# akanazawa/human_dynamics

Hardware: NVIDIA H100
Metric: frames/sec (ResNet->f_movie->SMPL LBS) (higher is better)
Workload: dtype f32 (wgmma 3x fp16 head/remainder split, fp32 two-level accumulate)

## Files before the change

human_dynamics_b200/_lib.py:

```python
from __future__ import annotations

import ctypes as C
import os

_HERE = os.path.dirname(os.path.abspath(__file__))
LIB_PATH = os.path.join(_HERE, 'libhd_b200.so')

HD_IMPL_SIMT, HD_IMPL_TC_3XTF32, HD_IMPL_TC_1XTF32, HD_IMPL_TC_3XF16, HD_IMPL_TC_1XF16 = 0, 1, 2, 3, 4
HD_CONV_NO_TMA_EPILOGUE = 1
HD_CONV_INPUT_PLANES = 2
HD_PACK_FORWARD, HD_PACK_BACKWARD_DATA = 0, 1
IMPL_BY_NAME = {'simt': HD_IMPL_SIMT, 'tc3': HD_IMPL_TC_3XTF32, 'tc1': HD_IMPL_TC_1XTF32, 'tc3h': HD_IMPL_TC_3XF16,
                'tc1h': HD_IMPL_TC_1XF16}


class ConvDesc(C.Structure):
    _fields_ = [
        ('in_', C.c_void_p), ('in_ld', C.c_longlong),
        ('n_img', C.c_int), ('H', C.c_int), ('W', C.c_int), ('Cin', C.c_int),
        ('Ho', C.c_int), ('Wo', C.c_int), ('KH', C.c_int), ('KW', C.c_int),
        ('stride', C.c_int), ('pad_t', C.c_int), ('pad_l', C.c_int),
        ('w_kn', C.c_void_p), ('w_nk_hi', C.c_void_p), ('w_nk_lo', C.c_void_p),
        ('Cout', C.c_int), ('K_pad', C.c_int),
        ('pre_scale', C.c_void_p), ('pre_shift', C.c_void_p), ('pre_img_stride', C.c_int), ('pre_relu', C.c_int),
        ('post_scale', C.c_void_p), ('post_shift', C.c_void_p), ('post_relu', C.c_int),
        ('res', C.c_void_p), ('res_ld', C.c_longlong), ('res_H', C.c_int), ('res_W', C.c_int), ('res_stride', C.c_int),
        ('out', C.c_void_p), ('out_ld', C.c_longlong),
        ('impl', C.c_int),
        ('tmap_hi', C.c_void_p), ('tmap_lo', C.c_void_p),
        ('in_hi', C.c_void_p), ('in_lo', C.c_void_p),
        ('out_hi', C.c_void_p), ('out_lo', C.c_void_p), ('out2_ld', C.c_longlong),
        ('post2_scale', C.c_void_p), ('post2_shift', C.c_void_p), ('post2_relu', C.c_int),
        ('tmap_res', C.c_void_p), ('tmap_out', C.c_void_p), ('tmap_out_hi', C.c_void_p), ('tmap_out_lo', C.c_void_p),
        ('flags', C.c_int),
        ('tmap_hi_n64', C.c_void_p), ('tmap_lo_n64', C.c_void_p),
        ('out_subsample', C.c_int),
    ]


WEIGHT_FN = C.CFUNCTYPE(C.c_void_p, C.c_void_p, C.c_char_p, C.POINTER(C.c_longlong))


class SmplConsts(C.Structure):
    _fields_ = [
        ('num_verts', C.c_int), ('num_kps', C.c_int), ('lbs_nnz', C.c_int), ('kp_nnz_total', C.c_int),
        ('v_template', C.c_void_p), ('dirs', C.c_void_p), ('J_template', C.c_void_p), ('J_shapedirs', C.c_void_p),
        ('lbs_idx', C.c_void_p), ('lbs_w', C.c_void_p),
        ('kp_ptr', C.c_void_p), ('kp_vidx', C.c_void_p), ('kp_w', C.c_void_p),
        ('parents', C.c_int * 24),
    ]


class SmplGradConsts(C.Structure):
    _fields_ = [
        ('num_verts', C.c_int), ('num_kps', C.c_int), ('num_tiles', C.c_int), ('tile_verts', C.c_int),
        ('kpv_ptr', C.c_void_p), ('kpv_kidx', C.c_void_p), ('kpv_w', C.c_void_p),
        ('lbt_ptr', C.c_void_p), ('lbt_v', C.c_void_p), ('lbt_w', C.c_void_p),
    ]


SMPL_GRAD_TILE, SMPL_GRAD_CLD = 256, 224


class RenderParams(C.Structure):
    _fields_ = [
        ('color', C.c_float * 3), ('light_dir', C.c_float * 3), ('ambient', C.c_float), ('directional', C.c_float),
        ('bg', C.c_float * 3), ('near_z', C.c_float), ('far_z', C.c_float), ('eye_z', C.c_float),
        ('rot', C.c_float * 9), ('use_rot', C.c_int),
    ]


HD_LOSS_KP_L1, HD_LOSS_MSE_ROWS = 0, 1
HD_LOSS_KP_CAMERA, HD_LOSS_KP_OPTCAM, HD_LOSS_KP_RAW = 0, 1, 2
HD_LOSS_MAX_TERMS, HD_LOSS_MAX_GRADS = 64, 16


class LossTerm(C.Structure):
    _fields_ = [
        ('kind', C.c_int), ('proj', C.c_int), ('B', C.c_int), ('Tw', C.c_int), ('p_t0', C.c_int), ('q_t0', C.c_int),
        ('p_T', C.c_int), ('q_T', C.c_int), ('K', C.c_int), ('D', C.c_int),
        ('p', C.c_void_p), ('p_clip', C.c_longlong), ('p_frame', C.c_longlong),
        ('q', C.c_void_p), ('q_clip', C.c_longlong), ('q_frame', C.c_longlong),
        ('cam', C.c_void_p), ('cam_clip', C.c_longlong), ('cam_frame', C.c_longlong),
        ('w', C.c_void_p), ('cam_out', C.c_void_p), ('scale', C.c_float),
    ]


class LossGrad(C.Structure):
    _fields_ = [('src', C.c_void_p), ('grad', C.c_void_p), ('numel', C.c_longlong)]


HD_ADAM_MAX_TENSORS = 256


class AdamTensor(C.Structure):
    _fields_ = [('param', C.c_void_p), ('grad', C.c_void_p), ('m', C.c_void_p), ('v', C.c_void_p), ('numel', C.c_longlong)]


HD_AUG_SRC_U8, HD_AUG_ROTATE, HD_AUG_FLIP = 1, 2, 4


class TubeAugArgs(C.Structure):
    _fields_ = [
        ('frames', C.c_void_p), ('F', C.c_int), ('H', C.c_int), ('W', C.c_int), ('flags', C.c_int),
        ('trans', C.c_void_p), ('scale', C.c_void_p), ('rot', C.c_void_p), ('flip', C.c_void_p),
        ('labels', C.c_void_p), ('K', C.c_int), ('centers', C.c_void_p), ('poses', C.c_void_p), ('gt3ds', C.c_void_p),
        ('S', C.c_int), ('trans_max', C.c_int), ('geom', C.c_void_p),
        ('labels_out', C.c_void_p), ('centers_out', C.c_void_p), ('poses_out', C.c_void_p), ('gt3ds_out', C.c_void_p),
        ('crops', C.c_void_p), ('plane_hi', C.c_void_p), ('plane_lo', C.c_void_p), ('WP', C.c_int),
    ]


HD_EVAL_KP, HD_EVAL_KP_PA, HD_EVAL_KP_PCK, HD_EVAL_JOINTS, HD_EVAL_JOINTS_PA, HD_EVAL_ACCEL, HD_EVAL_ACCEL_ERROR, HD_EVAL_VIS3D = range(8)
HD_EVAL_COLS = 8


class EvalFramesArgs(C.Structure):
    _fields_ = [
        ('N', C.c_int), ('n_seq', C.c_int), ('seq_start', C.c_void_p), ('K', C.c_int), ('J', C.c_int),
        ('kps_gt', C.c_void_p), ('kps_gt_ld', C.c_longlong), ('kps_pred', C.c_void_p), ('kps_pred_ld', C.c_longlong),
        ('joints_gt', C.c_void_p), ('joints_gt_ld', C.c_longlong), ('joints_pred', C.c_void_p), ('joints_pred_ld', C.c_longlong),
        ('img_size', C.c_float), ('min_visible', C.c_int), ('out', C.c_void_p),
    ]


HD_JPEG_BAD_CODE, HD_JPEG_OVERRUN, HD_JPEG_MARKER, HD_JPEG_BAD_HEADER = 1, 2, 4, 8


class JpegHuffman(C.Structure):
    _fields_ = [('bits', C.c_uint8 * 16), ('vals', C.c_uint8 * 256)]


class JpegHeader(C.Structure):
    _fields_ = [
        ('width', C.c_int), ('height', C.c_int), ('h_samp', C.c_int), ('v_samp', C.c_int), ('restart_interval', C.c_int),
        ('qt', C.c_int * 3), ('dc', C.c_int * 3), ('ac', C.c_int * 3), ('data_offset', C.c_longlong), ('data_bytes', C.c_longlong),
    ]


class JpegTables(C.Structure):
    _fields_ = [('quant', (C.c_uint16 * 64) * 4), ('dc', JpegHuffman * 4), ('ac', JpegHuffman * 4),
                ('quant_defined', C.c_int), ('dc_defined', C.c_int), ('ac_defined', C.c_int)]


_vp, _i, _ll, _f, _sz, _ull = C.c_void_p, C.c_int, C.c_longlong, C.c_float, C.c_size_t, C.c_ulonglong
SIGNATURES = {
    'hd_version': (_i, []),
    'hd_status_string': (C.c_char_p, [_i]),
    'hd_last_error': (C.c_char_p, []),
    'hd_launch_count': (_ll, []),
    'hd_launch_count_reset': (None, []),
    'hd_conv_gemm': (_i, [C.POINTER(ConvDesc), _vp]),
    'hd_conv_gemm_profile': (_i, [C.POINTER(ConvDesc), _vp, _vp]),
    'hd_conv_gemm_chain': (_i, [C.POINTER(ConvDesc), C.POINTER(ConvDesc), _vp]),
    'hd_conv_gemm_chain_supported': (_i, [C.POINTER(ConvDesc), C.POINTER(ConvDesc)]),
    'hd_make_weight_tmap': (_i, [_vp, _i, _i, _i, _i, _vp]),
    'hd_make_act_tmap': (_i, [_vp, _ll, _i, _ll, _i, _vp]),
    'hd_pack_conv1_planes': (_i, [_vp, _vp, _vp, _i, _i, _i, _i, _vp]),
    'hd_conv1_7x7s2': (_i, [_vp, _vp, _vp, _vp, _i, _i, _i, _vp]),
    'hd_maxpool3x3s2_same': (_i, [_vp, _vp, _i, _i, _i, _i, _vp, _vp, _vp, _vp, _vp]),
    'hd_subsample': (_i, [_vp, _vp, _i, _i, _i, _i, _i, _vp]),
    'hd_bnrelu_avgpool': (_i, [_vp, _vp, _vp, _vp, _i, _i, _i, _vp]),
    'hd_bn_stats_workspace_bytes': (_sz, [_ll, _i]),
    'hd_bn_batch_stats': (_i, [_vp, _ll, _i, _ll, _vp, _vp, _f] + [_vp] * 6 + [C.c_double, _vp, _sz, _vp]),
    'hd_bn_moving_update': (_i, [_vp, _vp, _ll, _i, C.c_double, _vp, _vp, _vp]),
    'hd_conv_wgrad_workspace_bytes': (_sz, [_ll, _i, _i, _i]),
    'hd_conv_wgrad': (_i, [_vp, _ll] + [_i] * 11 + [_vp, _vp, _vp, _ll, _i, _vp, _vp, _vp, _sz, _vp]),
    'hd_conv_wgrad_ex': (_i, [_vp, _ll] + [_i] * 11 + [_vp, _vp, _vp, _ll, _i, _vp, _vp, _vp, _sz, _i, _vp]),
    'hd_bn_relu_backward_workspace_bytes': (_sz, [_ll, _i]),
    'hd_bn_relu_backward': (_i, [_vp, _vp, _i, _ll, _i, _vp, _vp, _vp, _vp, _f, _vp, _i, _i, _i, _vp, _vp, _vp, _vp, _sz, _vp]),
    'hd_maxpool3x3s2_same_backward': (_i, [_vp, _vp, _vp, _i, _i, _i, _i, _vp]),
    'hd_zero_insert': (_i, [_vp, _vp] + [_i] * 7 + [_vp]),
    'hd_process_image': (_i, [_vp, _i, _i, _i, _vp, _vp, _i, _vp, _vp, _i, _vp]),
    'hd_crop_geometry': (_i, [_i, _i, _vp, _i, _vp, _vp, _vp]),
    'hd_groupnorm_stats': (_i, [_vp, _vp, _vp, _vp, _vp, _i, _i, _i, _i, _f, _vp]),
    'hd_groupnorm_relu_split': (_i, [_vp, _vp, _vp, _vp, _vp, _i, _i, _i, _i, _f, _vp]),
    'hd_split_f16': (_i, [_vp, _vp, _vp, _ll, _vp]),
    'hd_ief_fc1_theta': (_i, [_vp, _vp, _i, _vp, _i, _i, _vp, _vp, _vp, _i, _vp]),
    'hd_ief_fc3': (_i, [_vp, _vp, _vp, _vp, _i, _vp, _i, _i, _i, _i, _vp]),
    'hd_ief_fc1_theta_dropout': (_i, [_vp, _vp, _i, _vp, _i, _i, _vp, _vp, _vp, _i, _ull, _ull, _i, _f, _vp]),
    'hd_ief_fc3_dropout': (_i, [_vp, _vp, _vp, _vp, _i, _vp, _i, _i, _i, _i, _ull, _ull, _i, _f, _vp]),
    'hd_dropout_mask': (_i, [_ull, _ull, _i, _i, _i, _f, _vp, _vp]),
    'hd_ief_delta_init': (_i, [_vp, _vp, _i, _i, _vp]),
    'hd_net_destroy': (None, [_vp]),
    'hd_net_error': (C.c_char_p, [_vp]),
    'hd_net_num_launches': (_ll, [_vp]),
    'hd_resnet50_create': (_i, [_vp, _vp, _i, _i, C.POINTER(_vp)]),
    'hd_resnet50_forward': (_i, [_vp, _vp, _vp, _vp]),
    'hd_fmovie_create': (_i, [_vp, _vp, _i, _i, _i, C.POINTER(_vp)]),
    'hd_fmovie_forward': (_i, [_vp, _vp, _vp, _vp]),
    'hd_ief_create': (_i, [_vp, _vp, _i, C.POINTER(_i), _i, C.POINTER(_vp)]),
    'hd_ief_forward': (_i, [_vp, _vp, _vp, _vp, _vp]),
    'hd_smpl_pack_sizes': (_i, [_i, _i, _vp, _vp, C.POINTER(_i), C.POINTER(_i)]),
    'hd_smpl_pack': (_i, [_i, _i] + [_vp] * 13 + [_i] + [_vp] * 4),
    'hd_smpl_workspace_bytes': (_sz, [_i]),
    'hd_smpl_forward': (_i, [C.POINTER(SmplConsts), _vp, _i, _vp, _i, _i, _vp, _vp, _vp, _vp, _vp, _i, _vp, _i, _i, _vp, _sz, _vp]),
    'hd_smpl_pose': (_i, [C.POINTER(SmplConsts), _vp, _i, _vp, _i, _i, _vp, _vp, _vp, _vp, _i, _vp, _vp, _vp, _vp, _i, _i, _vp, _sz, _vp]),
    'hd_smpl_lbs_tc': (_i, [_vp, _vp, _vp, _vp, _vp, _ll, _vp, _i, _i, _i, _i, _vp]),
    'hd_smpl_lbs': (_i, [C.POINTER(SmplConsts), _vp, _ll, _vp, _vp, _i, _i, _i, _vp]),
    'hd_smpl_joints': (_i, [C.POINTER(SmplConsts), _vp, _vp, _i, _vp, _vp, _i, _i, _i, _vp]),
    'hd_rodrigues': (_i, [_vp, _vp, _i, _vp]),
    'hd_rot2aa': (_i, [_vp, _vp, _i, _vp]),
    'hd_global_rigid': (_i, [_vp, _vp, C.POINTER(C.c_int), _vp, _vp, _i, _i, _vp]),
    'hd_orth_proj': (_i, [_vp, _vp, _vp, _i, _i, _vp]),
    'hd_smpl_backward_workspace_bytes': (_sz, [_i, _i]),
    'hd_smpl_lbs_backward': (_i, [C.POINTER(SmplConsts), C.POINTER(SmplGradConsts), _vp, _ll, _vp, _vp, _vp, _vp, _vp, _i, _vp]),
    'hd_smpl_pose_backward': (_i, [C.POINTER(SmplConsts), _vp, _i, _vp, _i, _i, _vp, _vp, _i, _vp, _vp, _vp, _i, _vp, _i, _vp]),
    'hd_rodrigues_backward': (_i, [_vp, _vp, _vp, _i, _vp]),
    'hd_global_rigid_backward': (_i, [_vp, _vp, C.POINTER(C.c_int), _vp, _vp, _vp, _vp, _i, _i, _vp]),
    'hd_orth_proj_backward': (_i, [_vp, _vp, _vp, _vp, _vp, _i, _i, _vp]),
    'hd_pack_weight': (_i, [_vp, _i, _i, _i, _i, _i, _vp, _vp, _i, _i, _vp]),
    'hd_transpose_split': (_i, [_vp, _ll, _i, _ll, _i, _vp, _vp, _ll, _i, _ll, _vp]),
    'hd_im2col_t': (_i, [_vp, _i, _i, _i, _i, _i, _vp, _vp, _i, _vp, _ll, _ll, _vp]),
    'hd_groupnorm_relu_backward': (_i, [_vp] * 8 + [_i, _i, _i, _i, _f, _i, _vp]),
    'hd_col_sum': (_i, [_vp, _ll, _i, _ll, _vp, _vp]),
    'hd_relu_backward': (_i, [_vp, _vp, _vp, _ll, _vp]),
    'hd_fc_small_dgrad': (_i, [_vp, _i, _vp, _i, _i, _vp, _vp, _i, _vp]),
    'hd_relu_dropout_backward': (_i, [_vp, _vp, _vp, _ll, _f, _vp]),
    'hd_fc_small_dgrad_dropout': (_i, [_vp, _i, _vp, _i, _i, _vp, _f, _vp, _i, _vp]),
    'hd_add_strided': (_i, [_vp, _ll, _vp, _ll, _vp, _ll, _i, _i, _vp]),
    'hd_dpose_workspace_bytes': (_sz, [_i]),
    'hd_dpose_trunk_forward': (_i, [_vp] * 10 + [_i, _vp]),
    'hd_dpose_out_forward': (_i, [_vp] * 4 + [_i, _vp]),
    'hd_dpose_trunk_backward': (_i, [_vp] * 11 + [_sz, _i, _vp]),
    'hd_dpose_grad_reduce': (_i, [_vp, _sz, _i, _vp, _vp]),
    'hd_loss_workspace_bytes': (_sz, [_vp, _i]),
    'hd_loss_forward': (_i, [_vp, _i, _vp, _vp, _sz, _vp]),
    'hd_loss_backward': (_i, [_vp, _i, _vp, _i, _vp, _vp, _sz, _vp]),
    'hd_adam_tf': (_i, [C.POINTER(AdamTensor), _i, _f, _f, _f, _f, _vp, _vp]),
    'hd_render_workspace_bytes': (_sz, [_i, _i, _i]),
    'hd_tube_augment': (_i, [C.POINTER(TubeAugArgs), _vp]),
    'hd_render_mesh': (_i, [_vp, _ll, _i, _i, _vp, _i, _vp, _i, C.POINTER(RenderParams), _vp, _i, _vp, _vp, _vp, _sz, _vp]),
    'hd_eval_frames': (_i, [C.POINTER(EvalFramesArgs), _vp]),
    'hd_eval_mesh_tpose': (_i, [C.POINTER(SmplConsts), _vp, _i, _vp, _i, _i, _vp, _vp]),
    'hd_eval_verts_error': (_i, [_vp, _ll, _vp, _ll, _i, _i, _vp, _vp]),
    'hd_jpeg_parse': (_i, [_vp, _sz, C.POINTER(JpegHeader), C.POINTER(JpegTables)]),
    'hd_jpeg_workspace_bytes': (_sz, [_i, _i, _i, _i, _i]),
    'hd_jpeg_decode': (_i, [_vp, _ll, _vp, _i, _i, _i, _i, _i, _vp, _i, _vp, _i, _vp, _vp, _vp, _sz, _vp]),
}


def _load():
    if not os.path.exists(LIB_PATH):
        raise RuntimeError(
            'human_dynamics_b200: %s is missing -- build it with `make -C human_dynamics_b200/csrc` '
            '(or `python -c "import __graft_entry__ as g; g.build()"`). There is no CPU fallback.' % LIB_PATH)
    lib = C.CDLL(LIB_PATH)
    for name, (res, args) in SIGNATURES.items():
        fn = getattr(lib, name)
        fn.restype = res
        fn.argtypes = args
    return lib


lib = _load()


class HDError(RuntimeError):
    pass


def check(rc: int, what: str = ''):
    if rc != 0:
        raise HDError('%s failed: %s [%s]' % (what or 'libhd_b200 call', lib.hd_status_string(rc).decode(),
                                              lib.hd_last_error().decode()))


def dptr(t, dtype=None):
    import torch
    if t is None:
        return None
    if not isinstance(t, torch.Tensor) or not t.is_cuda:
        raise HDError('expected a CUDA torch.Tensor (no CPU fallback exists), got %r' % (type(t),))
    if dtype is not None and t.dtype != dtype:
        raise HDError('expected dtype %s, got %s' % (dtype, t.dtype))
    return C.c_void_p(t.data_ptr())


def fptr(t):
    import torch
    return dptr(t, torch.float32)


def current_stream():
    import torch
    return C.c_void_p(torch.cuda.current_stream().cuda_stream)
```

human_dynamics_b200/csrc/conv_tc.cu:

```cuda
#include <cuda.h>
#include <cuda_fp16.h>
#include <cstdlib>
#include "conv_common.cuh"
#include "tc_ptx.cuh"

namespace hd {
namespace {

constexpr int BM = 128;
constexpr int BOX_BYTES = 64 * 128;
constexpr int W_PROD = 8;
constexpr int STAGE_OUT = 1, STAGE_PAIR = 2;

using namespace ptx;

template <bool SPLIT, bool HALF, bool ASPLIT, int BN, bool RES = false, bool SHORT = false, bool CM = false>
struct Cfg {
  static_assert(BN == 64 || (BN == 128 && HALF && ASPLIT), "128-wide N tiles: pre-split fp16 path only");
  static_assert(!RES || ASPLIT, "residual by TMA: pre-split fp16 path only");
  static_assert(!SHORT || (BN == 64 && HALF && ASPLIT), "two CTAs per SM: 64-wide pre-split fp16 tiles only");
  static_assert(!CM || (BN == 64 && HALF && ASPLIT && !RES && !SHORT), "channels on M: 64-channel pre-split fp16 tiles, no residual");
  static constexpr int CTAS = SHORT ? 2 : 1;
  static constexpr int TM = CM ? 256 : BM;
  static constexpr int A_BYTES = TM * 128;
  static constexpr int PROD_THREADS = BN == 128 || SHORT || CM ? 128 : 256;
  static constexpr int NUM_THREADS = 256 + PROD_THREADS;
  static constexpr int ROW_STEP = PROD_THREADS / 8;
  static constexpr int ROWS = TM / ROW_STEP;
  static constexpr int PROD_REGS = SHORT ? 32 : CM ? 56 : BN == 128 ? 40 : 104, CONS_REGS = SHORT ? 104 : CM ? 224 : BN == 128 ? 232 : 152;
  static_assert(256 * CONS_REGS + PROD_THREADS * PROD_REGS <= NUM_THREADS * (65536 / (CTAS * NUM_THREADS) / 8 * 8),
                "setmaxnreg split beyond the CTA's registers");
  static constexpr int NACC = CM ? 64 : BN / 2;
  static constexpr int STAGES = SHORT ? 1 : CM ? 2 : BN == 128 ? (RES ? 2 : 3) : (RES ? 3 : 4);
  static constexpr int BKE = HALF ? 64 : 32;
  static constexpr int B_TILE_BYTES = BN * 128;
  static constexpr int B_OFFSET = (SPLIT ? 2 : 1) * A_BYTES;
  static constexpr int STAGE_BYTES = (SPLIT ? 2 : 1) * (A_BYTES + B_TILE_BYTES);
  static constexpr int RES_OFFSET = STAGES * STAGE_BYTES;
  static constexpr int RES_SLOT_BYTES = RES || SHORT ? 64 * BN * 4 : 0;
  static constexpr int STG_OFFSET = SHORT ? RES_OFFSET : RES_OFFSET + 2 * RES_SLOT_BYTES;
  static constexpr int STG_BYTES = ASPLIT ? (CM ? 4 : 2) * BOX_BYTES : 0;
  static_assert(!SHORT || STG_BYTES == RES_SLOT_BYTES, "SHORT: the staging buffer is the residual slot");
  static constexpr int BAR_OFFSET = SHORT ? RES_OFFSET + 2 * RES_SLOT_BYTES : STG_OFFSET + 2 * STG_BYTES;
  static constexpr int SMEM_BYTES = BAR_OFFSET + 128 + 1024;
  static_assert(SMEM_BYTES <= 232448, "dynamic shared memory beyond the 227 KB a CTA can opt into");
  static_assert(CTAS * (SMEM_BYTES + 1024) <= 233472, "CTAS CTAs (and the 1 KB each reserves) beyond an SM's 228 KB");
  static constexpr int PF = HALF ? 2 : 3;
  static constexpr int V = HALF ? 2 : 1;
};

template <bool ADD_R = false>
__device__ __forceinline__ void epi2_rn(float &y0, float &y1, const float *has_sc, float2 sc, const float *has_sh, float2 sh,
                                        const float2 *r, int relu) {
  if (has_sc) { y0 = __fmul_rn(y0, sc.x); y1 = __fmul_rn(y1, sc.y); }
  if (has_sh) { y0 = __fadd_rn(y0, sh.x); y1 = __fadd_rn(y1, sh.y); }
  if (ADD_R) { const float2 v = *r; y0 = __fadd_rn(y0, v.x); y1 = __fadd_rn(y1, v.y); }
  if (relu) { y0 = fmaxf(y0, 0.f); y1 = fmaxf(y1, 0.f); }
}

template <int R>
struct RowState {
  int n[R], iy[R], ix[R];
};

template <bool SPLIT, int PCH, bool HALF, bool GATHER, bool ASPLIT, int BN, bool RES, bool SHORT, bool CM>
__global__ void __launch_bounds__((Cfg<SPLIT, HALF, ASPLIT, BN, RES, SHORT, CM>::NUM_THREADS), (Cfg<SPLIT, HALF, ASPLIT, BN, RES, SHORT, CM>::CTAS))
conv_gemm_tc_kernel(const ConvParams p, const __grid_constant__ CUtensorMap tmap_hi, const __grid_constant__ CUtensorMap tmap_lo,
                    const __grid_constant__ CUtensorMap tmap_res, const __grid_constant__ CUtensorMap tmap_out,
                    const __grid_constant__ CUtensorMap tmap_out_hi, const __grid_constant__ CUtensorMap tmap_out_lo, const int stage) {
  using C = Cfg<SPLIT, HALF, ASPLIT, BN, RES, SHORT, CM>;
  constexpr bool MEM_STAMPS = BN == 128 || SHORT || CM;
  constexpr int BKE = C::BKE, PF = C::PF, V = C::V, STAGES = C::STAGES, R = C::ROWS, RS = C::ROW_STEP, NA = C::NACC;
  extern __shared__ uint8_t smem_raw[];
  const uint32_t smem_base = (smem_u32(smem_raw) + 1023u) & ~1023u;
  uint8_t *smem = smem_raw + (smem_base - smem_u32(smem_raw));
  const uint32_t bar_base = smem_base + C::BAR_OFFSET;
  auto full_bar = [&](int s) { return bar_base + 8u * s; };
  auto empty_bar = [&](int s) { return bar_base + 8u * (STAGES + s); };
  auto res_bar = [&](int g) { return bar_base + 8u * (2 * STAGES + g); };

  const int warp = threadIdx.x >> 5, lane = threadIdx.x & 31;
  const int num_k = (GATHER ? p.K_pad : p.K) / BKE;
  const int tiles_n = (p.Cout + BN - 1) / BN;
  const int num_tiles = ((p.M + C::TM - 1) / C::TM) * tiles_n;
  const int my_tiles = (num_tiles - (int)blockIdx.x + (int)gridDim.x - 1) / (int)gridDim.x;

  if (threadIdx.x == 0) {
    for (int s = 0; s < STAGES; ++s) {
      mbar_init(full_bar(s), ASPLIT ? C::PROD_THREADS + 1 : 9);
      mbar_init(empty_bar(s), 8);
    }
    if (RES) for (int g = 0; g < 2; ++g) mbar_init(res_bar(g), 1);
    asm volatile("fence.mbarrier_init.release.cluster;" ::: "memory");
  }
  __syncthreads();

  if (warp >= W_PROD) {
    asm volatile("setmaxnreg.dec.sync.aligned.u32 %0;" ::"n"(C::PROD_REGS));
    const int t = threadIdx.x - W_PROD * 32;
    const int j = t & 7;
    const int rb = t >> 3;
    const uint32_t sw_off = (uint32_t)((j ^ (rb & 7)) << 4);
    const bool prof = p.dbg != nullptr && blockIdx.x == 0 && t == 0;
    long long t_wait = 0, t_start = prof && !MEM_STAMPS ? clock64() : 0;
    if (MEM_STAMPS && prof) { p.dbg[0] = clock64(); p.dbg[1] = 0; }
    auto wait_empty = [&](int s, uint32_t ph) {
      if (MEM_STAMPS && prof) p.dbg[1] -= clock64();
      const long long tw0 = !MEM_STAMPS && prof ? clock64() : 0;
      mbar_wait(empty_bar(s), ph ^ 1u);
      if (!MEM_STAMPS && prof) t_wait += clock64() - tw0;
      if (MEM_STAMPS && prof) p.dbg[1] += clock64();
    };
    const int total = my_tiles * num_k;
    auto load_b = [&](int s, int ti, int kc) {
      if (t != 0) return;
      const int n0 = (((int)blockIdx.x + ti * (int)gridDim.x) % tiles_n) * BN;
      const uint32_t b_hi = smem_base + s * C::STAGE_BYTES + C::B_OFFSET;
      const int boxes = (BN == 128 && n0 + 64 < p.Cout) ? 2 : 1;
      mbar_arrive_expect_tx(full_bar(s), (SPLIT ? 2 : 1) * boxes * BOX_BYTES);
      for (int b = 0; b < boxes; ++b) {
        tma_load_2d(b_hi + b * BOX_BYTES, &tmap_hi, full_bar(s), kc * BKE, n0 + 64 * b);
        if (SPLIT) tma_load_2d(b_hi + C::B_TILE_BYTES + b * BOX_BYTES, &tmap_lo, full_bar(s), kc * BKE, n0 + 64 * b);
      }
    };

    auto enter_tile = [&](int ti, RowState<R> &rs) {
      const int tile = (int)blockIdx.x + ti * (int)gridDim.x;
      const int m0 = (tile / tiles_n) * C::TM;
      const int hw = p.Ho * p.Wo;
#pragma unroll
      for (int i = 0; i < R; ++i) {
        const int m = m0 + rb + RS * i;
        if (m < p.M) {
          const int n = m / hw;
          const int r = m - n * hw;
          const int oy = r / p.Wo, ox = r - oy * p.Wo;
          rs.n[i] = n; rs.iy[i] = oy * p.stride - p.pad_t; rs.ix[i] = ox * p.stride - p.pad_l;
        } else {
          rs.n[i] = -1; rs.iy[i] = 0; rs.ix[i] = 0;
        }
      }
    };
    if constexpr (ASPLIT) {
      const __half *ihi = reinterpret_cast<const __half *>(p.in_hi);
      const __half *ilo = reinterpret_cast<const __half *>(p.in_lo);
      if (SHORT || (!CM && !p.planes && p.KH * p.KW <= 32 && (long long)p.n_img * p.H * p.W * p.in_ld < (1ll << 31))) {
        const uint32_t off0 = (uint32_t)rb * 128u + sw_off;
        int base[R];
        uint32_t mask[R];
        int kc = 0, ti = 0, tap = 0, ci0 = 0, kx = 0, ky = 0, tap_off = 0;
        for (int q = 0; q < total; ++q) {
          if (kc == 0) {
            const int tile = (int)blockIdx.x + ti * (int)gridDim.x;
            const int m0 = (tile / tiles_n) * C::TM + rb;
            const int hw = p.Ho * p.Wo;
#pragma unroll
            for (int i = 0; i < R; ++i) {
              const int m = m0 + RS * i;
              uint32_t mk = 0;
              int b = 0;
              if (m < p.M) {
                const int n = m / hw;
                const int r = m - n * hw;
                const int oy = r / p.Wo, ox = r - oy * p.Wo;
                const int iy0 = oy * p.stride - p.pad_t, ix0 = ox * p.stride - p.pad_l;
                b = ((n * p.H + iy0) * p.W + ix0) * p.in_ld + j * 8;
                int t = 0;
                for (int yy = 0; yy < p.KH; ++yy)
                  for (int xx = 0; xx < p.KW; ++xx, ++t)
                    if ((unsigned)(iy0 + yy) < (unsigned)p.H && (unsigned)(ix0 + xx) < (unsigned)p.W) mk |= 1u << t;
              }
              base[i] = SHORT && !(mk & 1u) ? -1 : b;
              mask[i] = mk;
            }
            tap = 0; ci0 = 0; kx = 0; ky = 0; tap_off = 0;
          }
          const int s = q % STAGES;
          const uint32_t ph = (uint32_t)(q / STAGES) & 1u;
          wait_empty(s, ph);
          load_b(s, ti, kc);
          const uint32_t a_hi = smem_base + s * C::STAGE_BYTES + off0;
          const int eo = SHORT ? ci0 : tap_off + ci0;
#pragma unroll
          for (int i = 0; i < R; ++i) {
            const bool ok = SHORT ? base[i] >= 0 : (mask[i] >> tap) & 1u;
            const int e = ok ? base[i] + eo : 0;
            cp_async16(a_hi + i * RS * 128, ihi + e, ok ? 16u : 0u);
            if (SPLIT) cp_async16(a_hi + C::A_BYTES + i * RS * 128, ilo + e, ok ? 16u : 0u);
          }
          asm volatile("cp.async.mbarrier.arrive.noinc.shared::cta.b64 [%0];" ::"r"(full_bar(s)) : "memory");
          ci0 += BKE;
          if (ci0 == p.Cin) {
            ci0 = 0; ++tap;
            if (++kx == p.KW) { kx = 0; ++ky; }
            tap_off = (ky * p.W + kx) * p.in_ld;
          }
          if (++kc == num_k) { kc = 0; ++ti; }
        }
      } else if (!SHORT && p.planes && (long long)p.n_img * p.H * p.W * p.in_ld < (1ll << 31)) {
        const uint32_t off0 = (uint32_t)rb * 128u + sw_off;
        const int jt = j >> 2;
        const int row_step = 2 * p.W * (int)p.in_ld;
        int base[R];
        int kc = 0, ti = 0;
        for (int q = 0; q < total; ++q) {
          if (kc == 0) {
            const int tile = (int)blockIdx.x + ti * (int)gridDim.x;
            const int m0 = (tile / tiles_n) * C::TM + rb;
            const int hw = p.Ho * p.Wo;
#pragma unroll
            for (int i = 0; i < R; ++i) {
              const int m = m0 + RS * i;
              int b = -1;
              if (m < p.M) {
                const int n = m / hw;
                const int r = m - n * hw;
                const int oy = r / p.Wo, ox = r - oy * p.Wo;
                b = ((n * p.H + oy * p.stride + jt) * p.W + ox * p.stride) * (int)p.in_ld + (j & 3) * 8;
              }
              base[i] = b;
            }
          }
          const int s = q % STAGES;
          const uint32_t ph = (uint32_t)(q / STAGES) & 1u;
          wait_empty(s, ph);
          load_b(s, ti, kc);
          const uint32_t a_hi = smem_base + s * C::STAGE_BYTES + off0;
          const bool tap_ok = 2 * kc + jt < 7;
          const int eo = kc * row_step;
#pragma unroll
          for (int i = 0; i < R; ++i) {
            const bool ok = tap_ok && base[i] >= 0;
            const int e = ok ? base[i] + eo : 0;
            cp_async16_ca(a_hi + i * RS * 128, ihi + e, ok ? 16u : 0u);
            if (SPLIT) cp_async16_ca(a_hi + C::A_BYTES + i * RS * 128, ilo + e, ok ? 16u : 0u);
          }
          asm volatile("cp.async.mbarrier.arrive.noinc.shared::cta.b64 [%0];" ::"r"(full_bar(s)) : "memory");
          if (++kc == num_k) { kc = 0; ++ti; }
        }
      } else if (!SHORT && !CM) {
      RowState<R> rs;
      int kc = 0, ti = 0;
      for (int q = 0; q < total; ++q) {
        if (kc == 0) enter_tile(ti, rs);
        const int s = q % STAGES;
        const uint32_t ph = (uint32_t)(q / STAGES) & 1u;
        wait_empty(s, ph);
        load_b(s, ti, kc);
        const int kb = kc * BKE;
        const int tap = p.planes ? 2 * kc + (j >> 2) : kb / p.Cin;
        const int ci = p.planes ? (j & 3) * 8 : kb - tap * p.Cin + j * 8;
        const int ky = tap / p.KW, kx = tap - ky * p.KW;
        const bool tap_ok = !p.planes || tap < 7;
        const uint32_t a_hi = smem_base + s * C::STAGE_BYTES, a_lo = a_hi + C::A_BYTES;
#pragma unroll
        for (int i = 0; i < R; ++i) {
          const int iy = rs.iy[i] + ky, ix = rs.ix[i] + kx;
          const bool ok = tap_ok && rs.n[i] >= 0 && iy >= 0 && iy < p.H && ix >= 0 && ix < p.W;
          const size_t e = ok ? ((size_t)((size_t)rs.n[i] * p.H + iy) * p.W + ix) * p.in_ld + ci : 0;
          const uint32_t off = (uint32_t)(rb + RS * i) * 128u + sw_off;
          if (p.planes) {
            cp_async16_ca(a_hi + off, ihi + e, ok ? 16u : 0u);
            if (SPLIT) cp_async16_ca(a_lo + off, ilo + e, ok ? 16u : 0u);
          } else {
            cp_async16(a_hi + off, ihi + e, ok ? 16u : 0u);
            if (SPLIT) cp_async16(a_lo + off, ilo + e, ok ? 16u : 0u);
          }
        }
        asm volatile("cp.async.mbarrier.arrive.noinc.shared::cta.b64 [%0];" ::"r"(full_bar(s)) : "memory");
        if (++kc == num_k) { kc = 0; ++ti; }
      }
      }
      cp_async_commit();
      cp_async_wait<0>();
      if (prof) { p.dbg[0] = clock64() - (MEM_STAMPS ? p.dbg[0] : t_start); if (!MEM_STAMPS) p.dbg[1] = t_wait; }
    } else {
    RowState<R> pf_rs, st_rs;
    float4 ring[PF][4 * V];
    uint32_t vmask[PF];
    int pf_kc = 0, pf_ti = 0;
    auto prefetch = [&](float4 *dst, uint32_t &vm) {
      if (pf_kc == 0) enter_tile(pf_ti, pf_rs);
      if (GATHER) {
        const int seg = p.KW * p.Cin, segp = (seg + 7) & ~7;
        const int g8 = (pf_kc * BKE + j * (4 * V)) / 8;
        const int gpr = segp >> 3;
        const int ky = g8 / gpr, r0 = (g8 - ky * gpr) * 8;
        vm = 0;
#pragma unroll
        for (int i = 0; i < 4; ++i) {
          const int iy = pf_rs.iy[i] + ky;
          const bool okr = pf_rs.n[i] >= 0 && ky < p.KH && iy >= 0 && iy < p.H;
          const int c0 = pf_rs.ix[i] * p.Cin + r0;
          const float *src = p.in + ((size_t)((size_t)(okr ? pf_rs.n[i] : 0) * p.H + (okr ? iy : 0)) * p.W) * p.in_ld + c0;
          const int rowlen = p.W * p.Cin;
          float xs[8];
#pragma unroll
          for (int e = 0; e < 8; ++e) {
            const bool ok = okr && (r0 + e) < seg && (c0 + e) >= 0 && (c0 + e) < rowlen;
            xs[e] = ok ? __ldg(src + e) : 0.f;
          }
          dst[i * V] = make_float4(xs[0], xs[1], xs[2], xs[3]);
          dst[i * V + V - 1] = make_float4(xs[4], xs[5], xs[6], xs[7]);
          if (pf_rs.n[i] >= 0) vm |= 1u << i;
        }
        if (++pf_kc == num_k) { pf_kc = 0; ++pf_ti; }
        return;
      }
      const int kb = pf_kc * BKE;
      const int tap = kb / p.Cin, ci = kb - tap * p.Cin + j * (4 * V);
      const int ky = tap / p.KW, kx = tap - ky * p.KW;
      vm = 0;
#pragma unroll
      for (int i = 0; i < 4; ++i) {
        const int iy = pf_rs.iy[i] + ky, ix = pf_rs.ix[i] + kx;
        const bool ok = pf_rs.n[i] >= 0 && (unsigned)iy < (unsigned)p.H && (unsigned)ix < (unsigned)p.W;
        if (ok) {
          const float4 *src = reinterpret_cast<const float4 *>(p.in + ((size_t)((size_t)pf_rs.n[i] * p.H + iy) * p.W + ix) * p.in_ld + ci);
#pragma unroll
          for (int v = 0; v < V; ++v) dst[i * V + v] = __ldg(src + v);
          vm |= 1u << i;
        } else {
#pragma unroll
          for (int v = 0; v < V; ++v) dst[i * V + v] = make_float4(0.f, 0.f, 0.f, 0.f);
        }
      }
      if (++pf_kc == num_k) { pf_kc = 0; ++pf_ti; }
    };
    int st_kc = 0, st_ti = 0;
    auto consume = [&](int q, float4 *cur, uint32_t vm) {
      if (st_kc == 0) enter_tile(st_ti, st_rs);
      const int s = q % STAGES;
      const uint32_t ph = (uint32_t)(q / STAGES) & 1u;
      long long tw0 = prof ? clock64() : 0;
      mbar_wait(empty_bar(s), ph ^ 1u);
      if (prof) t_wait += clock64() - tw0;
      load_b(s, st_ti, st_kc);
      uint8_t *a_hi = smem + s * C::STAGE_BYTES;
      uint8_t *a_lo = a_hi + C::A_BYTES;
      const int pci = p.pre_scale ? (st_kc * BKE) % p.Cin + j * (4 * V) : 0;
#pragma unroll
      for (int i = 0; i < 4; ++i) {
        float xs[4 * V];
#pragma unroll
        for (int v = 0; v < V; ++v) {
          const float4 x = cur[i * V + v];
          xs[4 * v] = x.x; xs[4 * v + 1] = x.y; xs[4 * v + 2] = x.z; xs[4 * v + 3] = x.w;
        }
        if (p.pre_scale && (vm & (1u << i))) {
          const size_t po = (size_t)(p.pre_img_stride != 0 ? st_rs.n[i] : 0) * p.pre_img_stride + pci;
#pragma unroll
          for (int v = 0; v < V; ++v) {
            const float4 sc = __ldg(reinterpret_cast<const float4 *>(p.pre_scale + po) + v);
            const float4 sh = __ldg(reinterpret_cast<const float4 *>(p.pre_shift + po) + v);
            xs[4 * v] = xs[4 * v] * sc.x + sh.x; xs[4 * v + 1] = xs[4 * v + 1] * sc.y + sh.y;
            xs[4 * v + 2] = xs[4 * v + 2] * sc.z + sh.z; xs[4 * v + 3] = xs[4 * v + 3] * sc.w + sh.w;
          }
          if (p.pre_relu) {
#pragma unroll
            for (int e = 0; e < 4 * V; ++e) xs[e] = fmaxf(xs[e], 0.f);
          }
        }
        uint32_t h[4], l[4];
        if (!HALF) {
#pragma unroll
          for (int e = 0; e < 4; ++e) {
            const float hf = rn_tf32(xs[e]);
            h[e] = __float_as_uint(hf);
            l[e] = __float_as_uint(rn_tf32(xs[e] - hf));
          }
        } else {
#pragma unroll
          for (int e = 0; e < 4; ++e) split_f16x2(xs[2 * e], xs[2 * e + 1], h[e], l[e]);
        }
        const uint32_t off = (uint32_t)(rb + 32 * i) * 128u + sw_off;
        *reinterpret_cast<uint4 *>(a_hi + off) = make_uint4(h[0], h[1], h[2], h[3]);
        if (SPLIT) *reinterpret_cast<uint4 *>(a_lo + off) = make_uint4(l[0], l[1], l[2], l[3]);
      }
      asm volatile("fence.proxy.async.shared::cta;" ::: "memory");
      __syncwarp();
      if (lane == 0) mbar_arrive(full_bar(s));
      if (++st_kc == num_k) { st_kc = 0; ++st_ti; }
    };
#pragma unroll
    for (int u = 0; u < PF - 1; ++u)
      if (u < total) prefetch(ring[u], vmask[u]);
    for (int q0 = 0; q0 < total; q0 += PF) {
#pragma unroll
      for (int u = 0; u < PF; ++u) {
        const int q = q0 + u;
        if (q < total) {
          if (q + PF - 1 < total) prefetch(ring[(u + PF - 1) % PF], vmask[(u + PF - 1) % PF]);
          consume(q, ring[u], vmask[u]);
        }
      }
    }
    if (prof) { p.dbg[0] = clock64() - t_start; p.dbg[1] = t_wait; }
    }
  } else if (warp < W_PROD) {
    asm volatile("setmaxnreg.inc.sync.aligned.u32 %0;" ::"n"(C::CONS_REGS));
    const int wg = warp >> 2;
    const bool prof = p.dbg != nullptr && blockIdx.x == 0 && threadIdx.x == 0;
    long long t_wait = 0, t_start = prof && !MEM_STAMPS && !RES ? clock64() : 0;
    if ((RES || MEM_STAMPS) && prof) p.dbg[2] = clock64();
    if (prof) { p.dbg[3] = 0; p.dbg[4] = 0; p.dbg[5] = 0; p.dbg[6] = 0; }
    const int hw = p.Ho * p.Wo;
    const int frow = wg * 64 + (warp & 3) * 16 + (lane >> 2);
    const int fcol = 2 * (lane & 3);
    float acc[NA], accx[SPLIT ? NA : 1], sums_[SHORT ? 1 : NA];
    float *const sums = SHORT ? acc : sums_;
#pragma unroll
    for (int i = 0; i < NA; ++i) {
      acc[i] = 0.f;
      if constexpr (SPLIT) accx[i] = 0.f;
    }
    uint8_t *res_sm = smem + C::RES_OFFSET + wg * C::RES_SLOT_BYTES;
    const bool res_issuer = RES && (threadIdx.x & 127) == 0;
    const bool stg_issuer = ASPLIT && (threadIdx.x & 127) == 0;
    auto load_res = [&](int ti) {
      const int tile = (int)blockIdx.x + ti * (int)gridDim.x;
      const int r0 = (tile / tiles_n) * BM + 64 * wg, c0 = (tile % tiles_n) * BN;
      const int cols = p.Cout - c0 < BN ? p.Cout - c0 : BN;
      const int boxes = r0 < p.M ? (cols + 31) / 32 : 0;
      const uint32_t slot = smem_base + C::RES_OFFSET + wg * C::RES_SLOT_BYTES;
      mbar_arrive_expect_tx(res_bar(wg), boxes * (64 * 128));
      for (int b = 0; b < boxes; ++b) tma_load_2d(slot + b * (64 * 128), &tmap_res, res_bar(wg), c0 + 32 * b, r0);
    };
    if (res_issuer && my_tiles > 0) load_res(0);
    int q = 0;
    for (int ti = 0; ti < my_tiles; ++ti) {
      if (!SHORT) {
#pragma unroll
        for (int i = 0; i < NA; ++i) sums[i] = 0.f;
      }
      for (int kc = 0; kc < num_k; ++kc, ++q) {
        const int s = q % STAGES;
        const uint32_t ph = (uint32_t)(q / STAGES) & 1u;
        const bool group_start = (kc % PCH) == 0;
        if (MEM_STAMPS && prof) p.dbg[3] -= clock64();
        const long long tw0 = !MEM_STAMPS && prof ? clock64() : 0;
        mbar_wait(full_bar(s), ph);
        if (!MEM_STAMPS && prof) t_wait += clock64() - tw0;
        if (MEM_STAMPS && prof) p.dbg[3] += clock64();
        if (ASPLIT) asm volatile("fence.proxy.async.shared::cta;" ::: "memory");
        const uint32_t a_hi = smem_base + s * C::STAGE_BYTES + wg * (C::TM / 2 * 128);
        const uint32_t a_lo = a_hi + C::A_BYTES;
        const uint32_t b_hi = smem_base + s * C::STAGE_BYTES + C::B_OFFSET;
        const uint32_t b_lo = b_hi + C::B_TILE_BYTES;
        const uint64_t da_hi = make_smem_desc(a_hi), da_lo = make_smem_desc(a_lo);
        const uint64_t db_hi = make_smem_desc(b_hi), db_lo = make_smem_desc(b_lo);
        fence_regs(acc);
        if constexpr (SPLIT) fence_regs(accx);
        wgmma_fence();
#pragma unroll
        for (int k = 0; k < 4; ++k) {
          const uint64_t adv = (uint64_t)((k * 32) >> 4);
          if constexpr (CM) {
            if constexpr (SPLIT) {
              wgmma_m64n128k16_f16(accx, db_hi + adv, da_lo + adv, (kc | k) != 0);
              wgmma_m64n128k16_f16(accx, db_lo + adv, da_hi + adv, 1u);
            }
            wgmma_m64n128k16_f16(acc, db_hi + adv, da_hi + adv, !(group_start && k == 0));
          } else if constexpr (BN == 128) {
            if constexpr (SPLIT) {
              wgmma_m64n128k16_f16(accx, da_lo + adv, db_hi + adv, (kc | k) != 0);
              wgmma_m64n128k16_f16(accx, da_hi + adv, db_lo + adv, 1u);
            }
            wgmma_m64n128k16_f16(acc, da_hi + adv, db_hi + adv, !(group_start && k == 0));
          } else if constexpr (HALF) {
            if constexpr (SPLIT) {
              wgmma_m64n64k16_f16(accx, da_lo + adv, db_hi + adv, (kc | k) != 0);
              wgmma_m64n64k16_f16(accx, da_hi + adv, db_lo + adv, 1u);
            }
            wgmma_m64n64k16_f16(acc, da_hi + adv, db_hi + adv, !(group_start && k == 0));
          } else {
            if constexpr (SPLIT) {
              wgmma_m64n64k8_tf32(accx, da_lo + adv, db_hi + adv, (kc | k) != 0);
              wgmma_m64n64k8_tf32(accx, da_hi + adv, db_lo + adv, 1u);
            }
            wgmma_m64n64k8_tf32(acc, da_hi + adv, db_hi + adv, !(group_start && k == 0));
          }
        }
        wgmma_commit();
        wgmma_wait<0>();
        fence_regs(acc);
        if constexpr (SPLIT) fence_regs(accx);
        __syncwarp();
        if (lane == 0) mbar_arrive(empty_bar(s));
        if (!SHORT && ((kc % PCH) == PCH - 1 || kc == num_k - 1)) {
#pragma unroll
          for (int i = 0; i < NA; ++i) sums[i] += acc[i];
        }
      }
      if (SHORT) {
#pragma unroll
        for (int i = 0; i < NA; ++i) acc[i] = __fadd_rn(0.f, acc[i]);
      }
      if constexpr (SPLIT) {
#pragma unroll
        for (int i = 0; i < NA; ++i) sums[i] += accx[i] * (HALF ? (1.0f / 2048.0f) : 1.0f);
      }
      if (prof) p.dbg[4] -= clock64();
      const int tile = (int)blockIdx.x + ti * (int)gridDim.x;
      const int m0 = (tile / tiles_n) * C::TM, n0 = (tile % tiles_n) * BN;
      if (RES && prof) p.dbg[5] -= clock64();
      if (RES) mbar_wait(res_bar(wg), (uint32_t)ti & 1u);
      if (RES && prof) p.dbg[5] += clock64();
      auto row_geom = [&](int m, int &n_img, int &oy, int &ox) {
        n_img = 0; oy = 0; ox = 0;
        if (p.out_sub || (!RES && p.res && !(p.res_stride == 1 && p.res_H == p.Ho && p.res_W == p.Wo))) {
          n_img = m / hw;
          const int r = m - n_img * hw;
          oy = r / p.Wo; ox = r - oy * p.Wo;
        }
      };
      auto res_row = [&](int m, int n_img, int oy, int ox) -> const float * {
        if (RES || !p.res) return nullptr;
        const size_t rr = (p.res_stride == 1 && p.res_H == p.Ho && p.res_W == p.Wo)
                              ? (size_t)m
                              : ((size_t)n_img * p.res_H + (size_t)oy * p.res_stride) * p.res_W + (size_t)ox * p.res_stride;
        return p.res + rr * p.res_ld;
      };
      auto out_row = [&](int m, int n_img, int oy, int ox) -> float * {
        if (!p.out) return nullptr;
        if (!p.out_sub) return p.out + (size_t)m * p.out_ld;
        if (oy % p.out_sub != 0 || ox % p.out_sub != 0) return nullptr;
        const int Hs = (p.Ho + p.out_sub - 1) / p.out_sub, Ws = (p.Wo + p.out_sub - 1) / p.out_sub;
        return p.out + ((size_t)((size_t)n_img * Hs + oy / p.out_sub) * Ws + ox / p.out_sub) * p.out_ld;
      };
      auto value2 = [&](int c, const float2 *rs, const float *rrow, float &y0, float &y1) {
        if (p.post_scale) { const float2 sc = __ldg(reinterpret_cast<const float2 *>(p.post_scale + c)); y0 *= sc.x; y1 *= sc.y; }
        if (p.post_shift) { const float2 sh = __ldg(reinterpret_cast<const float2 *>(p.post_shift + c)); y0 += sh.x; y1 += sh.y; }
        if (RES) { const float2 r = *rs; y0 += r.x; y1 += r.y; }
        else if (rrow) { const float2 r = *reinterpret_cast<const float2 *>(rrow + c); y0 += r.x; y1 += r.y; }
        if (p.post_relu) { y0 = fmaxf(y0, 0.f); y1 = fmaxf(y1, 0.f); }
      };
      auto pair2 = [&](int c, float a0, float a1, uint32_t &hh, uint32_t &ll) {
        if (p.post2_scale) { const float2 sc = __ldg(reinterpret_cast<const float2 *>(p.post2_scale + c)); a0 *= sc.x; a1 *= sc.y; }
        if (p.post2_shift) { const float2 sh = __ldg(reinterpret_cast<const float2 *>(p.post2_shift + c)); a0 += sh.x; a1 += sh.y; }
        if (p.post2_relu) { a0 = fmaxf(a0, 0.f); a1 = fmaxf(a1, 0.f); }
        split_f16x2(a0, a1, hh, ll);
      };
      if constexpr (CM) {
        const bool st32 = (stage & STAGE_OUT) != 0;
        uint8_t *stg = smem + C::STG_OFFSET + wg * C::STG_BYTES;
        const uint32_t stg_a = smem_base + C::STG_OFFSET + wg * C::STG_BYTES;
        const int r0 = m0 + 128 * wg;
        const int ch = (warp & 3) * 16 + (lane >> 2);
        auto acquire = [&]() {
          if (prof) p.dbg[6] -= clock64();
          if (stg_issuer) bulk_wait_read<0>();
          named_bar_sync(3 + wg, 128);
          if (prof) p.dbg[6] += clock64();
        };
        if (st32) {
          acquire();
#pragma unroll
          for (int h = 0; h < 2; ++h) {
            const int c = ch + 8 * h;
            const float sc = p.post_scale ? __ldg(p.post_scale + c) : 0.f, sh = p.post_shift ? __ldg(p.post_shift + c) : 0.f;
            uint8_t *cb = stg + (c >> 5) * BOX_BYTES + (c & 3) * 4;
#pragma unroll
            for (int j = 0; j < 16; ++j) {
#pragma unroll
              for (int e = 0; e < 2; ++e) {
                const int r = 8 * (j & 7) + fcol + e;
                float y = sums[4 * j + 2 * h + e];
                if (p.post_scale) y = __fmul_rn(y, sc);
                if (p.post_shift) y = __fadd_rn(y, sh);
                if (p.post_relu) y = fmaxf(y, 0.f);
                *reinterpret_cast<float *>(cb + (j >> 3) * 2 * BOX_BYTES + r * 128 + ((((c & 31) >> 2) ^ (fcol + e)) << 4)) = y;
                sums[4 * j + 2 * h + e] = y;
              }
            }
          }
          fence_proxy_async();
          named_bar_sync(3 + wg, 128);
          if (stg_issuer) {
#pragma unroll
            for (int b = 0; b < 4; ++b)
              if (r0 + 64 * (b >> 1) < p.M) tma_store_2d(&tmap_out, stg_a + b * BOX_BYTES, 32 * (b & 1), r0 + 64 * (b >> 1));
            bulk_commit();
          }
        }
      } else if constexpr (ASPLIT) {
        const bool st32 = (stage & STAGE_OUT) != 0, st2 = (stage & STAGE_PAIR) != 0;
        uint8_t *stg = smem + C::STG_OFFSET + wg * C::STG_BYTES;
        const uint32_t stg_a = smem_base + C::STG_OFFSET + wg * C::STG_BYTES;
        const int r0 = m0 + 64 * wg;
        const uint32_t rsw = (uint32_t)(lane >> 2);
        auto acquire = [&](bool after_out) {
          if (prof) p.dbg[6] -= clock64();
          if (stg_issuer) {
            if (after_out) bulk_wait_read<1>();
            else bulk_wait_read<0>();
          }
          named_bar_sync(3 + wg, 128);
          if (prof) p.dbg[6] += clock64();
        };
#pragma unroll
        for (int cc = 0; cc < BN / 64; ++cc) {
          const int c0 = n0 + 64 * cc;
          const bool issue = stg_issuer && r0 < p.M && c0 < p.Cout;
          if (st32 && !RES) acquire(false);
          const bool rok[2] = {m0 + frow < p.M, m0 + frow + 8 < p.M};
          if (!RES && !st32 && st2 && !p.out && !p.res) {
            acquire(false);
            uint8_t *brow = stg + (frow - 64 * wg) * 128 + 4 * (lane & 3);
            const float *vsc = p.post_scale ? p.post_scale + c0 + fcol : nullptr, *vsh = p.post_shift ? p.post_shift + c0 + fcol : nullptr;
            const float *v2sc = p.post2_scale ? p.post2_scale + c0 + fcol : nullptr, *v2sh = p.post2_shift ? p.post2_shift + c0 + fcol : nullptr;
#pragma unroll
            for (int jj = 0; jj < 8; ++jj) {
              const int j = 8 * cc + jj;
              if (c0 + 8 * jj + fcol >= p.Cout) continue;
              const float2 sc = vsc ? __ldg(reinterpret_cast<const float2 *>(vsc + 8 * jj)) : make_float2(0.f, 0.f);
              const float2 sh = vsh ? __ldg(reinterpret_cast<const float2 *>(vsh + 8 * jj)) : make_float2(0.f, 0.f);
              const float2 sc2 = v2sc ? __ldg(reinterpret_cast<const float2 *>(v2sc + 8 * jj)) : make_float2(0.f, 0.f);
              const float2 sh2 = v2sh ? __ldg(reinterpret_cast<const float2 *>(v2sh + 8 * jj)) : make_float2(0.f, 0.f);
#pragma unroll
              for (int h = 0; h < 2; ++h) {
                if (!rok[h]) continue;
                float a0 = sums[4 * j + 2 * h], a1 = sums[4 * j + 2 * h + 1];
                epi2_rn(a0, a1, vsc, sc, vsh, sh, nullptr, p.post_relu);
                epi2_rn(a0, a1, v2sc, sc2, v2sh, sh2, nullptr, p.post2_relu);
                uint32_t hh, ll;
                split_f16x2(a0, a1, hh, ll);
                uint32_t *hs = reinterpret_cast<uint32_t *>(brow + h * 1024 + (((uint32_t)jj ^ rsw) * 16));
                hs[0] = hh;
                if (SPLIT) hs[BOX_BYTES / 4] = ll;
              }
            }
            fence_proxy_async();
            named_bar_sync(3 + wg, 128);
            if (issue) {
              tma_store_2d(&tmap_out_hi, stg_a, c0, r0);
              if (SPLIT) tma_store_2d(&tmap_out_lo, stg_a + BOX_BYTES, c0, r0);
            }
            if (stg_issuer) bulk_commit();
            continue;
          }
          if (st32 && (RES || !p.res)) {
            uint8_t *brow = (RES ? res_sm + 2 * cc * BOX_BYTES : stg) + (frow - 64 * wg) * 128 + 8 * (lane & 1);
            const float *vsc = p.post_scale ? p.post_scale + c0 + fcol : nullptr, *vsh = p.post_shift ? p.post_shift + c0 + fcol : nullptr;
#pragma unroll
            for (int jj = 0; jj < 8; ++jj) {
              const int j = 8 * cc + jj;
              if (c0 + 8 * jj + fcol >= p.Cout) continue;
              const uint32_t piece = (uint32_t)(2 * (jj & 3) + ((lane & 3) >> 1)) ^ rsw;
              const float2 sc = vsc ? __ldg(reinterpret_cast<const float2 *>(vsc + 8 * jj)) : make_float2(0.f, 0.f);
              const float2 sh = vsh ? __ldg(reinterpret_cast<const float2 *>(vsh + 8 * jj)) : make_float2(0.f, 0.f);
#pragma unroll
              for (int h = 0; h < 2; ++h) {
                if (!rok[h]) continue;
                float2 *f32 = reinterpret_cast<float2 *>(brow + h * 1024 + (jj >> 2) * BOX_BYTES + piece * 16);
                float y0 = sums[4 * j + 2 * h], y1 = sums[4 * j + 2 * h + 1];
                epi2_rn<RES>(y0, y1, vsc, sc, vsh, sh, f32, p.post_relu);
                *f32 = make_float2(y0, y1);
                sums[4 * j + 2 * h] = y0; sums[4 * j + 2 * h + 1] = y1;
              }
            }
          } else {
#pragma unroll
          for (int h = 0; h < 2; ++h) {
            const int m = m0 + frow + 8 * h;
            if (m >= p.M) continue;
            int n_img, oy, ox;
            row_geom(m, n_img, oy, ox);
            const float *rrow = res_row(m, n_img, oy, ox);
            float *orow = st32 ? nullptr : out_row(m, n_img, oy, ox);
            uint8_t *brow = (RES ? res_sm + 2 * cc * BOX_BYTES : stg) + (frow - 64 * wg + 8 * h) * 128 + 8 * (lane & 1);
#pragma unroll
            for (int jj = 0; jj < 8; ++jj) {
              const int j = 8 * cc + jj;
              const int c = n0 + 8 * j + fcol;
              if (c >= p.Cout) continue;
              const uint32_t piece = (uint32_t)(2 * (jj & 3) + ((lane & 3) >> 1)) ^ rsw;
              float2 *f32 = reinterpret_cast<float2 *>(brow + (jj >> 2) * BOX_BYTES + piece * 16);
              float y0 = sums[4 * j + 2 * h], y1 = sums[4 * j + 2 * h + 1];
              value2(c, f32, rrow, y0, y1);
              if (st32) *f32 = make_float2(y0, y1);
              else if (orow) *reinterpret_cast<float2 *>(orow + c) = make_float2(y0, y1);
              sums[4 * j + 2 * h] = y0; sums[4 * j + 2 * h + 1] = y1;
            }
          }
          }
          if (st32) {
            fence_proxy_async();
            named_bar_sync(3 + wg, 128);
            if (issue) {
              const uint32_t src = RES ? smem_base + C::RES_OFFSET + wg * C::RES_SLOT_BYTES + 2 * cc * BOX_BYTES : stg_a;
              tma_store_2d(&tmap_out, src, c0, r0);
              if (c0 + 32 < p.Cout) tma_store_2d(&tmap_out, src + BOX_BYTES, c0 + 32, r0);
            }
            if (stg_issuer) bulk_commit();
          }
          if (p.out_hi) {
            if (st2) acquire(RES && st32 && !SHORT);
            if (st2) {
              uint8_t *brow = stg + (frow - 64 * wg) * 128 + 4 * (lane & 3);
              const float *vsc = p.post2_scale ? p.post2_scale + c0 + fcol : nullptr, *vsh = p.post2_shift ? p.post2_shift + c0 + fcol : nullptr;
#pragma unroll
              for (int jj = 0; jj < 8; ++jj) {
                const int j = 8 * cc + jj;
                if (c0 + 8 * jj + fcol >= p.Cout) continue;
                const float2 sc = vsc ? __ldg(reinterpret_cast<const float2 *>(vsc + 8 * jj)) : make_float2(0.f, 0.f);
                const float2 sh = vsh ? __ldg(reinterpret_cast<const float2 *>(vsh + 8 * jj)) : make_float2(0.f, 0.f);
#pragma unroll
                for (int h = 0; h < 2; ++h) {
                  if (!rok[h]) continue;
                  float a0 = sums[4 * j + 2 * h], a1 = sums[4 * j + 2 * h + 1];
                  epi2_rn(a0, a1, vsc, sc, vsh, sh, nullptr, p.post2_relu);
                  uint32_t hh, ll;
                  split_f16x2(a0, a1, hh, ll);
                  uint32_t *hs = reinterpret_cast<uint32_t *>(brow + h * 1024 + (((uint32_t)jj ^ rsw) * 16));
                  hs[0] = hh;
                  if (SPLIT) hs[BOX_BYTES / 4] = ll;
                }
              }
            } else {
#pragma unroll
            for (int h = 0; h < 2; ++h) {
              const int m = m0 + frow + 8 * h;
              if (m >= p.M) continue;
              __half *hrow = reinterpret_cast<__half *>(p.out_hi) + (size_t)m * p.out2_ld;
              __half *lrow = SPLIT ? reinterpret_cast<__half *>(p.out_lo) + (size_t)m * p.out2_ld : nullptr;
              uint8_t *brow = stg + (frow - 64 * wg + 8 * h) * 128 + 4 * (lane & 3);
#pragma unroll
              for (int jj = 0; jj < 8; ++jj) {
                const int j = 8 * cc + jj;
                const int c = n0 + 8 * j + fcol;
                if (c >= p.Cout) continue;
                uint32_t hh, ll;
                pair2(c, sums[4 * j + 2 * h], sums[4 * j + 2 * h + 1], hh, ll);
                if (st2) {
                  uint32_t *hs = reinterpret_cast<uint32_t *>(brow + (((uint32_t)jj ^ rsw) * 16));
                  hs[0] = hh;
                  if (SPLIT) hs[BOX_BYTES / 4] = ll;
                } else {
                  *reinterpret_cast<uint32_t *>(hrow + c) = hh;
                  if (SPLIT) *reinterpret_cast<uint32_t *>(lrow + c) = ll;
                }
              }
            }
            }
            if (st2) {
              fence_proxy_async();
              named_bar_sync(3 + wg, 128);
              if (issue) {
                tma_store_2d(&tmap_out_hi, stg_a, c0, r0);
                if (SPLIT) tma_store_2d(&tmap_out_lo, stg_a + BOX_BYTES, c0, r0);
              }
              if (stg_issuer) bulk_commit();
            }
          }
        }
      } else {
#pragma unroll
      for (int h = 0; h < 2; ++h) {
        const int m = m0 + frow + 8 * h;
        if (m >= p.M) continue;
        int n_img, oy, ox;
        row_geom(m, n_img, oy, ox);
        const float *rrow = res_row(m, n_img, oy, ox);
        float *orow = out_row(m, n_img, oy, ox);
        __half *hrow = p.out_hi ? reinterpret_cast<__half *>(p.out_hi) + (size_t)m * p.out2_ld : nullptr;
        __half *lrow = SPLIT && p.out_hi ? reinterpret_cast<__half *>(p.out_lo) + (size_t)m * p.out2_ld : nullptr;
#pragma unroll
        for (int j = 0; j < BN / 8; ++j) {
          const int c = n0 + 8 * j + fcol;
          if (c >= p.Cout) continue;
          const bool two = c + 1 < p.Cout;
          float y[2] = {sums[4 * j + 2 * h], sums[4 * j + 2 * h + 1]};
          if (p.vec_out) {
            value2(c, nullptr, rrow, y[0], y[1]);
            if (orow) *reinterpret_cast<float2 *>(orow + c) = make_float2(y[0], y[1]);
            if (hrow) {
              uint32_t hh, ll;
              pair2(c, y[0], y[1], hh, ll);
              *reinterpret_cast<uint32_t *>(hrow + c) = hh;
              if (SPLIT) *reinterpret_cast<uint32_t *>(lrow + c) = ll;
            }
          } else {
#pragma unroll
            for (int e = 0; e < 2; ++e) {
              if (e == 1 && !two) break;
              float v = y[e];
              if (p.post_scale) v *= __ldg(p.post_scale + c + e);
              if (p.post_shift) v += __ldg(p.post_shift + c + e);
              if (rrow) v += rrow[c + e];
              if (p.post_relu) v = fmaxf(v, 0.f);
              if (orow) orow[c + e] = v;
            }
          }
        }
      }
      }
      if (RES && ti + 1 < my_tiles) {
        if (prof) p.dbg[6] -= clock64();
        named_bar_sync(1 + wg, 128);
        if (res_issuer) {
          if (SHORT) {
            if (stage) bulk_wait_read<0>();
          } else if (stage & STAGE_OUT) {
            if (stage & STAGE_PAIR) bulk_wait_read<1>();
            else bulk_wait_read<0>();
          }
          load_res(ti + 1);
        }
        if (prof) p.dbg[6] += clock64();
      }
      if (prof) p.dbg[4] += clock64();
    }
    if (stg_issuer) bulk_wait_all();
    if (prof) { p.dbg[2] = clock64() - (RES || MEM_STAMPS ? p.dbg[2] : t_start); if (!MEM_STAMPS) p.dbg[3] = t_wait; }
    if (prof) { p.dbg[7] = C::TM; p.dbg[8] = BN; }
  }
}

template <bool SPLIT>
struct ChainCfg {
  static constexpr int NUM_THREADS = 384;
  static constexpr int SEGS = 4;
  static constexpr int A_BYTES = BM * 128;
  static constexpr int A_STAGE = (SPLIT ? 2 : 1) * A_BYTES;
  static constexpr int W1_OFFSET = (SPLIT ? 2 : 1) * BOX_BYTES;
  static constexpr int W_STAGE = 2 * W1_OFFSET;
  static constexpr int RES_SLOT = 64 * 64 * 4;
  static constexpr int PAIR_BYTES = 2 * BOX_BYTES;
  static constexpr int W_OFFSET = 2 * A_STAGE;
  static constexpr int RES_OFFSET = W_OFFSET + 2 * W_STAGE;
  static constexpr int PAIR_OFFSET = RES_OFFSET + 4 * RES_SLOT;
  static constexpr int BAR_OFFSET = PAIR_OFFSET + 2 * PAIR_BYTES;
  static constexpr int SMEM_BYTES = BAR_OFFSET + 128 + 1024;
  static_assert(SMEM_BYTES <= 232448, "dynamic shared memory beyond the 227 KB a CTA can opt into");
  static constexpr int PROD_REGS = 40, CONS_REGS = 232;
  static_assert(256 * CONS_REGS + 128 * PROD_REGS <= NUM_THREADS * (65536 / NUM_THREADS / 8 * 8), "setmaxnreg split beyond the CTA's registers");
};

template <bool SPLIT>
__global__ void __launch_bounds__(384, 1)
conv_chain_tc_kernel(const ConvParams p, const ConvParams q, const __grid_constant__ CUtensorMap tw3_hi,
                     const __grid_constant__ CUtensorMap tw3_lo, const __grid_constant__ CUtensorMap tw1_hi,
                     const __grid_constant__ CUtensorMap tw1_lo, const __grid_constant__ CUtensorMap tmap_res,
                     const __grid_constant__ CUtensorMap tmap_out, const __grid_constant__ CUtensorMap tmap_r1_hi,
                     const __grid_constant__ CUtensorMap tmap_r1_lo, const int st32) {
  using C = ChainCfg<SPLIT>;
  extern __shared__ uint8_t smem_raw[];
  const uint32_t smem_base = (smem_u32(smem_raw) + 1023u) & ~1023u;
  uint8_t *smem = smem_raw + (smem_base - smem_u32(smem_raw));
  const uint32_t bar_base = smem_base + C::BAR_OFFSET;
  auto full_a = [&](int s) { return bar_base + 8u * s; };
  auto empty_a = [&](int s) { return bar_base + 8u * (2 + s); };
  auto full_w = [&](int s) { return bar_base + 8u * (4 + s); };
  auto empty_w = [&](int s) { return bar_base + 8u * (6 + s); };
  auto res_bar = [&](int g, int e) { return bar_base + 8u * (8 + 2 * g + e); };
  const int warp = threadIdx.x >> 5, lane = threadIdx.x & 31;
  const int num_tiles = (p.M + BM - 1) / BM;
  const int my_tiles = (num_tiles - (int)blockIdx.x + (int)gridDim.x - 1) / (int)gridDim.x;

  if (threadIdx.x == 0) {
    for (int s = 0; s < 2; ++s) {
      mbar_init(full_a(s), 128);
      mbar_init(empty_a(s), 8);
      mbar_init(full_w(s), 1);
      mbar_init(empty_w(s), 8);
    }
    for (int i = 0; i < 4; ++i) mbar_init(bar_base + 8u * (8 + i), 1);
    asm volatile("fence.mbarrier_init.release.cluster;" ::: "memory");
  }
  __syncthreads();

  if (warp >= W_PROD) {
    asm volatile("setmaxnreg.dec.sync.aligned.u32 %0;" ::"n"(C::PROD_REGS));
    const int t = threadIdx.x - W_PROD * 32, j = t & 7, rb = t >> 3;
    const uint32_t off0 = (uint32_t)rb * 128u + (uint32_t)((j ^ (rb & 7)) << 4);
    const __half *ihi = reinterpret_cast<const __half *>(p.in_hi);
    const __half *ilo = reinterpret_cast<const __half *>(p.in_lo);
    int wq = 0;
    for (int ti = 0; ti < my_tiles; ++ti) {
      const int m0 = ((int)blockIdx.x + ti * (int)gridDim.x) * BM;
      const int sa = ti & 1;
      mbar_wait(empty_a(sa), ((uint32_t)(ti >> 1) & 1u) ^ 1u);
      const uint32_t a_hi = smem_base + sa * C::A_STAGE + off0;
#pragma unroll
      for (int i = 0; i < 8; ++i) {
        const int m = m0 + rb + 16 * i;
        const bool ok = m < p.M;
        const int e = ok ? m * (int)p.in_ld + j * 8 : 0;
        cp_async16(a_hi + i * 16 * 128, ihi + e, ok ? 16u : 0u);
        if (SPLIT) cp_async16(a_hi + C::A_BYTES + i * 16 * 128, ilo + e, ok ? 16u : 0u);
      }
      asm volatile("cp.async.mbarrier.arrive.noinc.shared::cta.b64 [%0];" ::"r"(full_a(sa)) : "memory");
      if (t == 0) {
        for (int s = 0; s < C::SEGS; ++s, ++wq) {
          const int sw = wq & 1;
          mbar_wait(empty_w(sw), ((uint32_t)(wq >> 1) & 1u) ^ 1u);
          mbar_arrive_expect_tx(full_w(sw), 2 * C::W1_OFFSET);
          const uint32_t wb = smem_base + C::W_OFFSET + sw * C::W_STAGE;
          tma_load_2d(wb, &tw3_hi, full_w(sw), 0, 64 * s);
          if (SPLIT) tma_load_2d(wb + BOX_BYTES, &tw3_lo, full_w(sw), 0, 64 * s);
          tma_load_2d(wb + C::W1_OFFSET, &tw1_hi, full_w(sw), 64 * s, 0);
          if (SPLIT) tma_load_2d(wb + C::W1_OFFSET + BOX_BYTES, &tw1_lo, full_w(sw), 64 * s, 0);
        }
      }
    }
    cp_async_commit();
    cp_async_wait<0>();
  } else {
    asm volatile("setmaxnreg.inc.sync.aligned.u32 %0;" ::"n"(C::CONS_REGS));
    const int wg = warp >> 2;
    const int frow = wg * 64 + (warp & 3) * 16 + (lane >> 2);
    const int fcol = 2 * (lane & 3);
    const uint32_t rsw = (uint32_t)(lane >> 2);
    const bool issuer = (threadIdx.x & 127) == 0;
    const uint32_t pb_a = smem_base + C::PAIR_OFFSET + wg * C::PAIR_BYTES;
    uint8_t *const pbrow = smem + C::PAIR_OFFSET + wg * C::PAIR_BYTES + (frow - 64 * wg) * 128 + 4 * (lane & 3);
    auto slot_a = [&](int e) { return smem_base + C::RES_OFFSET + (2 * wg + e) * C::RES_SLOT; };
    auto load_res = [&](int u) {
      if ((u >> 2) >= my_tiles) return;
      const int r0 = ((int)blockIdx.x + (u >> 2) * (int)gridDim.x) * BM + 64 * wg, c0 = 64 * (u & 3);
      const int boxes = r0 < p.M ? 2 : 0;
      mbar_arrive_expect_tx(res_bar(wg, u & 1), boxes * BOX_BYTES);
      for (int b = 0; b < boxes; ++b) tma_load_2d(slot_a(u & 1) + b * BOX_BYTES, &tmap_res, res_bar(wg, u & 1), c0 + 32 * b, r0);
    };
    if (issuer) { load_res(0); load_res(1); }
    float acc3[32], accx3[SPLIT ? 32 : 1], acc1[32], accx1[SPLIT ? 32 : 1], sums1[32];
    const int hw = p.Ho * p.Wo;
    int wq = 0;
    for (int ti = 0; ti < my_tiles; ++ti) {
      const int m0 = ((int)blockIdx.x + ti * (int)gridDim.x) * BM, r0 = m0 + 64 * wg;
      const bool rok[2] = {m0 + frow < p.M, m0 + frow + 8 < p.M};
      const int sa = ti & 1;
      mbar_wait(full_a(sa), (uint32_t)(ti >> 1) & 1u);
      asm volatile("fence.proxy.async.shared::cta;" ::: "memory");
      const uint32_t a_hi = smem_base + sa * C::A_STAGE + wg * 64 * 128;
      const uint64_t da_hi = make_smem_desc(a_hi), da_lo = make_smem_desc(a_hi + C::A_BYTES);
      const uint64_t dp_hi = make_smem_desc(pb_a), dp_lo = make_smem_desc(pb_a + BOX_BYTES);
#pragma unroll
      for (int i = 0; i < 32; ++i) sums1[i] = 0.f;
      for (int s = 0; s < C::SEGS; ++s, ++wq) {
        const int u = 4 * ti + s, e = u & 1, sw = wq & 1;
        mbar_wait(full_w(sw), (uint32_t)(wq >> 1) & 1u);
        const uint32_t wb = smem_base + C::W_OFFSET + sw * C::W_STAGE;
        const uint64_t d3_hi = make_smem_desc(wb), d3_lo = make_smem_desc(wb + BOX_BYTES);
        const uint64_t d1_hi = make_smem_desc(wb + C::W1_OFFSET), d1_lo = make_smem_desc(wb + C::W1_OFFSET + BOX_BYTES);
        fence_regs(acc3);
        if constexpr (SPLIT) fence_regs(accx3);
        wgmma_fence();
#pragma unroll
        for (int k = 0; k < 4; ++k) {
          const uint64_t adv = (uint64_t)((k * 32) >> 4);
          if constexpr (SPLIT) {
            wgmma_m64n64k16_f16(accx3, da_lo + adv, d3_hi + adv, k != 0);
            wgmma_m64n64k16_f16(accx3, da_hi + adv, d3_lo + adv, 1u);
          }
          wgmma_m64n64k16_f16(acc3, da_hi + adv, d3_hi + adv, k != 0);
        }
        wgmma_commit();
        wgmma_wait<0>();
        fence_regs(acc3);
        if constexpr (SPLIT) fence_regs(accx3);
        if (s == C::SEGS - 1) {
          __syncwarp();
          if (lane == 0) mbar_arrive(empty_a(sa));
        }
#pragma unroll
        for (int i = 0; i < 32; ++i) acc3[i] = __fadd_rn(0.f, acc3[i]);
        if constexpr (SPLIT) {
#pragma unroll
          for (int i = 0; i < 32; ++i) acc3[i] += accx3[i] * (1.0f / 2048.0f);
        }
        mbar_wait(res_bar(wg, e), (uint32_t)(u >> 1) & 1u);
        uint8_t *brow = smem + C::RES_OFFSET + (2 * wg + e) * C::RES_SLOT + (frow - 64 * wg) * 128 + 8 * (lane & 1);
        const float *vsh = p.post_shift ? p.post_shift + 64 * s + fcol : nullptr;
#pragma unroll
        for (int jj = 0; jj < 8; ++jj) {
          const uint32_t piece = (uint32_t)(2 * (jj & 3) + ((lane & 3) >> 1)) ^ rsw;
          const float2 sh = vsh ? __ldg(reinterpret_cast<const float2 *>(vsh + 8 * jj)) : make_float2(0.f, 0.f);
#pragma unroll
          for (int h = 0; h < 2; ++h) {
            if (!rok[h]) continue;
            float2 *f32 = reinterpret_cast<float2 *>(brow + h * 1024 + (jj >> 2) * BOX_BYTES + piece * 16);
            float y0 = acc3[4 * jj + 2 * h], y1 = acc3[4 * jj + 2 * h + 1];
            epi2_rn<true>(y0, y1, nullptr, make_float2(0.f, 0.f), vsh, sh, f32, 0);
            if (st32) *f32 = make_float2(y0, y1);
            acc3[4 * jj + 2 * h] = y0; acc3[4 * jj + 2 * h + 1] = y1;
          }
        }
        if (!st32) {
#pragma unroll
          for (int h = 0; h < 2; ++h) {
            const int m = m0 + frow + 8 * h;
            if (m >= p.M) continue;
            const int n_img = m / hw, r = m - n_img * hw, oy = r / p.Wo, ox = r - oy * p.Wo;
            if (oy % p.out_sub != 0 || ox % p.out_sub != 0) continue;
            const int Hs = (p.Ho + p.out_sub - 1) / p.out_sub, Ws = (p.Wo + p.out_sub - 1) / p.out_sub;
            float *orow = p.out + ((size_t)((size_t)n_img * Hs + oy / p.out_sub) * Ws + ox / p.out_sub) * p.out_ld + 64 * s + fcol;
#pragma unroll
            for (int jj = 0; jj < 8; ++jj)
              *reinterpret_cast<float2 *>(orow + 8 * jj) = make_float2(acc3[4 * jj + 2 * h], acc3[4 * jj + 2 * h + 1]);
          }
        }
        if (s == 0 && ti > 0) {
          if (issuer) bulk_wait_read<0>();
          named_bar_sync(1 + wg, 128);
        }
        {
          const float *v2sc = p.post2_scale ? p.post2_scale + 64 * s + fcol : nullptr, *v2sh = p.post2_shift ? p.post2_shift + 64 * s + fcol : nullptr;
#pragma unroll
          for (int jj = 0; jj < 8; ++jj) {
            const float2 sc2 = v2sc ? __ldg(reinterpret_cast<const float2 *>(v2sc + 8 * jj)) : make_float2(0.f, 0.f);
            const float2 sh2 = v2sh ? __ldg(reinterpret_cast<const float2 *>(v2sh + 8 * jj)) : make_float2(0.f, 0.f);
#pragma unroll
            for (int h = 0; h < 2; ++h) {
              float a0 = acc3[4 * jj + 2 * h], a1 = acc3[4 * jj + 2 * h + 1];
              epi2_rn(a0, a1, v2sc, sc2, v2sh, sh2, nullptr, p.post2_relu);
              uint32_t hh, ll;
              split_f16x2(a0, a1, hh, ll);
              uint32_t *hs = reinterpret_cast<uint32_t *>(pbrow + h * 1024 + (((uint32_t)jj ^ rsw) * 16));
              hs[0] = hh;
              if (SPLIT) hs[BOX_BYTES / 4] = ll;
            }
          }
        }
        fence_proxy_async();
        named_bar_sync(1 + wg, 128);
        if (issuer && st32) {
          if (r0 < p.M) {
            tma_store_2d(&tmap_out, slot_a(e), 64 * s, r0);
            tma_store_2d(&tmap_out, slot_a(e) + BOX_BYTES, 64 * s + 32, r0);
          }
          bulk_commit();
        }
        fence_regs(acc1);
        if constexpr (SPLIT) fence_regs(accx1);
        wgmma_fence();
#pragma unroll
        for (int k = 0; k < 4; ++k) {
          const uint64_t adv = (uint64_t)((k * 32) >> 4);
          if constexpr (SPLIT) {
            wgmma_m64n64k16_f16(accx1, dp_lo + adv, d1_hi + adv, (s | k) != 0);
            wgmma_m64n64k16_f16(accx1, dp_hi + adv, d1_lo + adv, 1u);
          }
          wgmma_m64n64k16_f16(acc1, dp_hi + adv, d1_hi + adv, !((s & 1) == 0 && k == 0));
        }
        wgmma_commit();
        if (issuer) {
          bulk_wait_read<0>();
          load_res(u + 2);
        }
        wgmma_wait<0>();
        fence_regs(acc1);
        if constexpr (SPLIT) fence_regs(accx1);
        __syncwarp();
        if (lane == 0) mbar_arrive(empty_w(sw));
        if (s & 1) {
#pragma unroll
          for (int i = 0; i < 32; ++i) sums1[i] += acc1[i];
        }
      }
      if constexpr (SPLIT) {
#pragma unroll
        for (int i = 0; i < 32; ++i) sums1[i] += accx1[i] * (1.0f / 2048.0f);
      }
      named_bar_sync(1 + wg, 128);
      {
        const float *vsc = q.post_scale ? q.post_scale + fcol : nullptr, *vsh = q.post_shift ? q.post_shift + fcol : nullptr;
        const float *v2sc = q.post2_scale ? q.post2_scale + fcol : nullptr, *v2sh = q.post2_shift ? q.post2_shift + fcol : nullptr;
#pragma unroll
        for (int jj = 0; jj < 8; ++jj) {
          const float2 sc = vsc ? __ldg(reinterpret_cast<const float2 *>(vsc + 8 * jj)) : make_float2(0.f, 0.f);
          const float2 sh = vsh ? __ldg(reinterpret_cast<const float2 *>(vsh + 8 * jj)) : make_float2(0.f, 0.f);
          const float2 sc2 = v2sc ? __ldg(reinterpret_cast<const float2 *>(v2sc + 8 * jj)) : make_float2(0.f, 0.f);
          const float2 sh2 = v2sh ? __ldg(reinterpret_cast<const float2 *>(v2sh + 8 * jj)) : make_float2(0.f, 0.f);
#pragma unroll
          for (int h = 0; h < 2; ++h) {
            float a0 = sums1[4 * jj + 2 * h], a1 = sums1[4 * jj + 2 * h + 1];
            epi2_rn(a0, a1, vsc, sc, vsh, sh, nullptr, q.post_relu);
            epi2_rn(a0, a1, v2sc, sc2, v2sh, sh2, nullptr, q.post2_relu);
            uint32_t hh, ll;
            split_f16x2(a0, a1, hh, ll);
            uint32_t *hs = reinterpret_cast<uint32_t *>(pbrow + h * 1024 + (((uint32_t)jj ^ rsw) * 16));
            hs[0] = hh;
            if (SPLIT) hs[BOX_BYTES / 4] = ll;
          }
        }
      }
      fence_proxy_async();
      named_bar_sync(1 + wg, 128);
      if (issuer) {
        if (r0 < p.M) {
          tma_store_2d(&tmap_r1_hi, pb_a, 0, r0);
          if (SPLIT) tma_store_2d(&tmap_r1_lo, pb_a + BOX_BYTES, 0, r0);
        }
        bulk_commit();
      }
    }
    if (issuer) bulk_wait_all();
  }
}

typedef CUresult (*EncodeTiledFn)(CUtensorMap *, CUtensorMapDataType, cuuint32_t, void *, const cuuint64_t *, const cuuint64_t *,
                                  const cuuint32_t *, const cuuint32_t *, CUtensorMapInterleave, CUtensorMapSwizzle,
                                  CUtensorMapL2promotion, CUtensorMapFloatOOBfill);

EncodeTiledFn get_encode_fn() {
  static EncodeTiledFn fn = nullptr;
  static bool tried = false;
  if (!tried) {
    tried = true;
    void *ptr = nullptr;
    cudaDriverEntryPointQueryResult qres;
    cudaError_t e = cudaGetDriverEntryPoint("cuTensorMapEncodeTiled", &ptr, cudaEnableDefault, &qres);
    if (e == cudaSuccess && qres == cudaDriverEntryPointSuccess) fn = reinterpret_cast<EncodeTiledFn>(ptr);
    else (void)cudaGetLastError();
  }
  return fn;
}

constexpr int kMaxDevices = 64;

int encode_epilogue_map(CUtensorMap *tm, bool fp16, const void *base, int cols, int rows, long long ld_bytes, const char *what) {
  EncodeTiledFn fn = get_encode_fn();
  if (!fn) { set_last_error_text("cuTensorMapEncodeTiled unavailable (no CUDA driver?)"); return HD_ERR_UNSUPPORTED; }
  const cuuint64_t gdim[2] = {(cuuint64_t)cols, (cuuint64_t)rows};
  const cuuint64_t gstride[1] = {(cuuint64_t)ld_bytes};
  const cuuint32_t box[2] = {fp16 ? 64u : 32u, 64u};
  const cuuint32_t estr[2] = {1u, 1u};
  CUresult r = fn(tm, fp16 ? CU_TENSOR_MAP_DATA_TYPE_FLOAT16 : CU_TENSOR_MAP_DATA_TYPE_FLOAT32, 2, const_cast<void *>(base), gdim, gstride,
                  box, estr, CU_TENSOR_MAP_INTERLEAVE_NONE, CU_TENSOR_MAP_SWIZZLE_128B, CU_TENSOR_MAP_L2_PROMOTION_L2_128B,
                  CU_TENSOR_MAP_FLOAT_OOB_FILL_NONE);
  if (r != CUDA_SUCCESS) {
    char msg[96];
    snprintf(msg, sizeof(msg), "cuTensorMapEncodeTiled (%s) failed with CUresult %d", what, (int)r);
    set_last_error_text(msg);
    return HD_ERR_CUDA;
  }
  return HD_OK;
}

template <bool SPLIT, int PCH, bool HALF, bool GATHER = false, bool ASPLIT = false, int BN = 64, bool RES = false, bool SHORT = false,
          bool CM = false>
int launch_tc(const ConvParams &p, const hd_conv_desc *d, cudaStream_t st) {
  using C = Cfg<SPLIT, HALF, ASPLIT, BN, RES, SHORT, CM>;
  static bool configured[kMaxDevices] = {};
  static int num_sms[kMaxDevices] = {};
  int dev = 0;
  cudaGetDevice(&dev);
  if (dev < 0 || dev >= kMaxDevices) { set_last_error_text("conv_gemm_tc: device ordinal out of range"); return HD_ERR_UNSUPPORTED; }
  if (!configured[dev]) {
    cudaError_t e = cudaFuncSetAttribute(conv_gemm_tc_kernel<SPLIT, PCH, HALF, GATHER, ASPLIT, BN, RES, SHORT, CM>,
                                         cudaFuncAttributeMaxDynamicSharedMemorySize, C::SMEM_BYTES);
    if (e != cudaSuccess) { set_last_error("conv_gemm_tc attr", e); return HD_ERR_CUDA; }
    cudaDeviceGetAttribute(&num_sms[dev], cudaDevAttrMultiProcessorCount, dev);
    if (num_sms[dev] <= 0) { set_last_error_text("conv_gemm_tc: no multiprocessor count"); return HD_ERR_CUDA; }
    configured[dev] = true;
  }
  alignas(64) CUtensorMap thi, tlo;
  const void *mhi = d->tmap_hi_n64 ? d->tmap_hi_n64 : d->tmap_hi;
  const void *mlo = d->tmap_hi_n64 ? d->tmap_lo_n64 : d->tmap_lo;
  memcpy(&thi, mhi, sizeof(CUtensorMap));
  memcpy(&tlo, mlo ? mlo : mhi, sizeof(CUtensorMap));
  alignas(64) CUtensorMap tres, tout, tohi, tolo;
  memcpy(&tres, &thi, sizeof(CUtensorMap));
  memcpy(&tout, &thi, sizeof(CUtensorMap));
  memcpy(&tohi, &thi, sizeof(CUtensorMap));
  memcpy(&tolo, &thi, sizeof(CUtensorMap));
  int rc = HD_OK;
  if (RES) rc = encode_epilogue_map(&tres, false, p.res, p.Cout, p.M, p.res_ld * 4, "residual");
  int stage = 0;
  if (ASPLIT && p.out && !p.out_sub) {
    stage |= STAGE_OUT;
    if (rc == HD_OK) rc = encode_epilogue_map(&tout, false, p.out, p.Cout, p.M, p.out_ld * 4, "output");
  }
  if (ASPLIT && p.out_hi && p.out2_ld % 8 == 0) {
    stage |= STAGE_PAIR;
    if (rc == HD_OK) rc = encode_epilogue_map(&tohi, true, p.out_hi, p.Cout, p.M, p.out2_ld * 2, "output head");
    if (rc == HD_OK && SPLIT) rc = encode_epilogue_map(&tolo, true, p.out_lo, p.Cout, p.M, p.out2_ld * 2, "output remainder");
  }
  if (rc != HD_OK) return rc;
  const int num_tiles = ceil_div(p.M, C::TM) * ceil_div(p.Cout, BN);
  const int ctas = C::CTAS * num_sms[dev];
  dim3 grid(num_tiles < ctas ? num_tiles : ctas);
  conv_gemm_tc_kernel<SPLIT, PCH, HALF, GATHER, ASPLIT, BN, RES, SHORT, CM>
      <<<grid, C::NUM_THREADS, C::SMEM_BYTES, st>>>(p, thi, tlo, tres, tout, tohi, tolo, stage);
  return check_launch("conv_gemm_tc_kernel");
}

bool wide_n_tile(const ConvParams &p) {
  if (p.Cout <= 64) return false;
  int dev = 0, sms = 0;
  cudaGetDevice(&dev);
  cudaDeviceGetAttribute(&sms, cudaDevAttrMultiProcessorCount, dev);
  if (sms <= 0) return true;
  const long long m_tiles = ceil_div(p.M, BM);
  const long long w128 = (m_tiles * ceil_div(p.Cout, 128) + sms - 1) / sms, w64 = (m_tiles * ceil_div(p.Cout, 64) + sms - 1) / sms;
  return 16 * w128 <= 9 * w64;
}


bool cout_on_m(const ConvParams &p) {
  if (!p.planes || p.Cout != 64 || p.res || p.out_sub || p.out_hi || !p.out) return false;
  if ((long long)p.n_img * p.H * p.W * p.in_ld >= (1ll << 31)) return false;
  int dev = 0, sms = 0;
  cudaGetDevice(&dev);
  cudaDeviceGetAttribute(&sms, cudaDevAttrMultiProcessorCount, dev);
  if (sms <= 0) return true;
  const long long w256 = (ceil_div(p.M, 256) + sms - 1) / sms, w128 = (ceil_div(p.M, BM) + sms - 1) / sms;
  return 16 * w256 <= 9 * w128;
}

template <bool SPLIT, bool RES>
bool short_k_two_ctas() {
  using C = Cfg<SPLIT, true, true, 64, RES, true>;
  static int two[kMaxDevices] = {};
  int dev = 0;
  cudaGetDevice(&dev);
  if (dev < 0 || dev >= kMaxDevices) return false;
  if (two[dev] == 0) {
    const auto kernel = conv_gemm_tc_kernel<SPLIT, 2, true, false, true, 64, RES, true, false>;
    int n = 0;
    if (cudaFuncSetAttribute(kernel, cudaFuncAttributeMaxDynamicSharedMemorySize, C::SMEM_BYTES) != cudaSuccess ||
        cudaOccupancyMaxActiveBlocksPerMultiprocessor(&n, kernel, C::NUM_THREADS, C::SMEM_BYTES) != cudaSuccess) {
      (void)cudaGetLastError();
      n = 0;
    }
    two[dev] = n >= 2 ? 1 : -1;
  }
  return two[dev] > 0;
}

template <bool SPLIT>
int launch_conv_f16(const ConvParams &p, const hd_conv_desc *d, cudaStream_t st) {
  if (p.in_hi && p.planes) {
    if (p.Cin != 32 || p.KH != 8 || p.KW != 1 || p.stride != 2 || p.pad_t != 0 || p.pad_l != 0 || p.in_ld != 4 || p.Cout > 64 ||
        p.W % 2 != 0 || 2 * (p.Wo - 1) + 8 > p.W || 2 * (p.Ho - 1) + 7 > p.H || !aligned16(p.in_hi) || !aligned16(p.in_lo) || p.pre_scale) {
      set_last_error_text("hd_conv_gemm(tc planes): needs the conv1 plane geometry (Cin 32, KH 8, KW 1, stride 2, in_ld 4, even W)");
      return HD_ERR_INVALID;
    }
    return cout_on_m(p) ? launch_tc<SPLIT, 2, true, false, true, 64, false, false, true>(p, d, st) : launch_tc<SPLIT, 2, true, false, true>(p, d, st);
  }
  if (p.in_hi) {
    if (p.Cin % 64 != 0 || p.K % 64 != 0 || p.in_ld % 8 != 0 || !aligned16(p.in_hi) || !aligned16(p.in_lo) || p.pre_scale) {
      set_last_error_text("hd_conv_gemm(tc split-A): needs Cin % 64 == 0, in_ld % 8 == 0, aligned in_hi/in_lo, no prologue");
      return HD_ERR_INVALID;
    }
    const bool res_rows = p.res && p.res_stride == 1 && p.res_H == p.Ho && p.res_W == p.Wo && p.K <= 8 * 64;
    const bool short_k = p.K <= 2 * 64 && p.KH * p.KW == 1 && (long long)p.n_img * p.H * p.W * p.in_ld < (1ll << 31) &&
                         (p.res ? res_rows : p.out_hi != nullptr);
    if (short_k && (res_rows ? short_k_two_ctas<SPLIT, true>() : short_k_two_ctas<SPLIT, false>()))
      return res_rows ? launch_tc<SPLIT, 2, true, false, true, 64, true, true>(p, d, st)
                      : launch_tc<SPLIT, 2, true, false, true, 64, false, true>(p, d, st);
    if (wide_n_tile(p))
      return res_rows ? launch_tc<SPLIT, 2, true, false, true, 128, true>(p, d, st) : launch_tc<SPLIT, 2, true, false, true, 128>(p, d, st);
    return res_rows ? launch_tc<SPLIT, 2, true, false, true, 64, true>(p, d, st) : launch_tc<SPLIT, 2, true, false, true>(p, d, st);
  }
  if (p.Cin % 64 != 0) {
    const int segp = (p.KW * p.Cin + 7) & ~7;
    if (p.K_pad % 64 != 0 || p.K_pad < p.KH * segp || p.Cout > 64 || p.pre_scale || p.in_ld != p.Cin) {
      set_last_error_text("hd_conv_gemm(tc gather): needs K_pad % 64 == 0, K_pad >= KH*roundup8(KW*Cin), Cout <= 64, dense pixels, no prologue");
      return HD_ERR_INVALID;
    }
    return launch_tc<SPLIT, 2, true, true>(p, d, st);
  }
  if (!p.in || p.in_ld % 4 != 0 || !aligned16(p.in) || p.K % 64 != 0 ||
      (p.pre_scale && (!aligned16(p.pre_scale) || !aligned16(p.pre_shift) || p.pre_img_stride % 4 != 0))) {
    set_last_error_text("hd_conv_gemm(tc): needs Cin % 32 (tf32) / % 64 (fp16) == 0 and 16-byte aligned input / prologue vectors");
    return HD_ERR_INVALID;
  }
  return launch_tc<SPLIT, 2, true>(p, d, st);
}

}

int launch_conv_tc(const ConvParams &p, const hd_conv_desc *d, cudaStream_t st) {
  const bool heads = d->impl == HD_IMPL_TC_1XF16;
  const bool split_b = d->impl != HD_IMPL_TC_1XTF32 && !heads;
  if (!d->tmap_hi || (split_b && !d->tmap_lo) || (!d->tmap_hi_n64 && d->tmap_lo_n64) || (d->tmap_hi_n64 && split_b && !d->tmap_lo_n64)) {
    set_last_error_text("hd_conv_gemm(tc): missing tensor maps (tmap_hi/tmap_lo, and tmap_hi_n64/tmap_lo_n64 together or not at all)");
    return HD_ERR_INVALID;
  }
  const bool half = d->impl == HD_IMPL_TC_3XF16 || heads;
  if (p.out_sub) {
    const bool res_plain = !p.res || (p.res_stride == 1 && p.res_H == p.Ho && p.res_W == p.Wo);
    const bool maps = (!p.res || d->tmap_res) && (!p.out_hi || (d->tmap_out_hi && (heads || d->tmap_out_lo)));
    if (!p.in_hi || p.planes || !maps || !res_plain || p.Cout % 32 != 0 || (d->flags & HD_CONV_NO_TMA_EPILOGUE)) {
      set_last_error_text("hd_conv_gemm: out_subsample needs the activation-map epilogue (pre-split input, Cout % 32 == 0, activation maps given)");
      return HD_ERR_UNSUPPORTED;
    }
  }
  if ((p.out_hi || p.in_hi) && (!half || !p.vec_out)) {
    set_last_error_text("hd_conv_gemm(tc): pre-split activations need impl 3 / 4 and 16-byte aligned, 4-column-multiple outputs");
    return HD_ERR_INVALID;
  }
  if (half) return heads ? launch_conv_f16<false>(p, d, st) : launch_conv_f16<true>(p, d, st);
  if (!p.in || p.Cin % 32 != 0 || p.in_ld % 4 != 0 || !aligned16(p.in) || p.K % 32 != 0 ||
      (p.pre_scale && (!aligned16(p.pre_scale) || !aligned16(p.pre_shift) || p.pre_img_stride % 4 != 0))) {
    set_last_error_text("hd_conv_gemm(tc): needs Cin % 32 (tf32) / % 64 (fp16) == 0 and 16-byte aligned input / prologue vectors");
    return HD_ERR_INVALID;
  }
  return d->impl != HD_IMPL_TC_1XTF32 ? launch_tc<true, 2, false>(p, d, st) : launch_tc<false, 8, false>(p, d, st);
}

int chain_check(const hd_conv_desc *a, const hd_conv_desc *b) {
  auto refuse = [](const char *why) {
    char msg[160];
    snprintf(msg, sizeof(msg), "hd_conv_gemm_chain: %s", why);
    set_last_error_text(msg);
    return HD_ERR_UNSUPPORTED;
  };
  if (!a || !b) return refuse("null descriptor");
  if (a->impl != b->impl || (a->impl != HD_IMPL_TC_3XF16 && a->impl != HD_IMPL_TC_1XF16)) return refuse("both convs need impl 3 or impl 4");
  const bool heads = a->impl == HD_IMPL_TC_1XF16;
  auto one_by_one = [heads](const hd_conv_desc *d) {
    return d->KH == 1 && d->KW == 1 && d->stride == 1 && d->pad_t == 0 && d->pad_l == 0 && d->Ho == d->H && d->Wo == d->W &&
           !d->pre_scale && !d->pre_shift && !(d->flags & HD_CONV_INPUT_PLANES) && d->K_pad == d->Cin && d->tmap_hi &&
           (heads ? !d->tmap_lo : d->tmap_lo != nullptr) && !d->tmap_hi_n64;
  };
  if (!one_by_one(a) || !one_by_one(b)) return refuse("both convs must be 1x1 stride 1 without prologue, with their weight maps");
  if (a->Cin != 64 || a->Cout != 256 || b->Cin != a->Cout || b->Cout != 64)
    return refuse("supported shape: conv3 64 -> 256 channels, then conv1 256 -> 64");
  if (!a->in_hi || (heads ? a->in_lo != nullptr : !a->in_lo) || a->in_ld % 8 != 0 || !aligned16(a->in_hi) || (a->in_lo && !aligned16(a->in_lo)) ||
      (long long)a->n_img * a->H * a->W * a->in_ld >= (1ll << 31))
    return refuse("the first conv reads an aligned pre-split pair with 32-bit element offsets");
  if (!a->res || a->res_stride != 1 || a->res_H != a->Ho || a->res_W != a->Wo || a->res_ld % 4 != 0 || !aligned16(a->res))
    return refuse("the first conv needs a row-aligned residual");
  if (!a->out || a->out_ld % 4 != 0 || !aligned16(a->out) || a->out_hi || a->out_lo || a->post_scale || a->post_relu ||
      (a->post_shift && !aligned16(a->post_shift)) || (a->post2_scale == nullptr) != (a->post2_shift == nullptr))
    return refuse("the first conv writes the fp32 output (or its subsample) and hands its post2 pair to the second");
  if (b->n_img != a->n_img || b->H != a->Ho || b->W != a->Wo || b->in || b->in_hi || b->in_lo || b->res || b->out ||
      b->out_subsample > 1 || !b->out_hi || (heads ? b->out_lo != nullptr : !b->out_lo) || b->out2_ld % 8 != 0 ||
      !aligned16(b->out_hi) || (b->out_lo && !aligned16(b->out_lo)))
    return refuse("the second conv reads the first's output rows and writes its pair alone");
  return HD_OK;
}

template <bool SPLIT>
int launch_chain(const ConvParams &p, const ConvParams &q, const hd_conv_desc *a, const hd_conv_desc *b, cudaStream_t st) {
  using C = ChainCfg<SPLIT>;
  static bool configured[kMaxDevices] = {};
  static int num_sms[kMaxDevices] = {};
  int dev = 0;
  cudaGetDevice(&dev);
  if (dev < 0 || dev >= kMaxDevices) { set_last_error_text("hd_conv_gemm_chain: device ordinal out of range"); return HD_ERR_UNSUPPORTED; }
  if (!configured[dev]) {
    cudaError_t e = cudaFuncSetAttribute(conv_chain_tc_kernel<SPLIT>, cudaFuncAttributeMaxDynamicSharedMemorySize, C::SMEM_BYTES);
    if (e != cudaSuccess) { set_last_error("hd_conv_gemm_chain attr", e); return HD_ERR_CUDA; }
    cudaDeviceGetAttribute(&num_sms[dev], cudaDevAttrMultiProcessorCount, dev);
    if (num_sms[dev] <= 0) { set_last_error_text("hd_conv_gemm_chain: no multiprocessor count"); return HD_ERR_CUDA; }
    configured[dev] = true;
  }
  alignas(64) CUtensorMap w3h, w3l, w1h, w1l, tres, tout, r1h, r1l;
  memcpy(&w3h, a->tmap_hi, sizeof(CUtensorMap));
  memcpy(&w3l, SPLIT ? a->tmap_lo : a->tmap_hi, sizeof(CUtensorMap));
  memcpy(&w1h, b->tmap_hi, sizeof(CUtensorMap));
  memcpy(&w1l, SPLIT ? b->tmap_lo : b->tmap_hi, sizeof(CUtensorMap));
  memcpy(&tout, &w3h, sizeof(CUtensorMap));
  memcpy(&r1l, &w3h, sizeof(CUtensorMap));
  const int st32 = p.out_sub ? 0 : 1;
  int rc = encode_epilogue_map(&tres, false, p.res, p.Cout, p.M, p.res_ld * 4, "residual");
  if (rc == HD_OK && st32) rc = encode_epilogue_map(&tout, false, p.out, p.Cout, p.M, p.out_ld * 4, "output");
  if (rc == HD_OK) rc = encode_epilogue_map(&r1h, true, q.out_hi, q.Cout, q.M, q.out2_ld * 2, "second output head");
  if (rc == HD_OK && SPLIT) rc = encode_epilogue_map(&r1l, true, q.out_lo, q.Cout, q.M, q.out2_ld * 2, "second output remainder");
  if (rc != HD_OK) return rc;
  const int num_tiles = ceil_div(p.M, BM);
  dim3 grid(num_tiles < num_sms[dev] ? num_tiles : num_sms[dev]);
  conv_chain_tc_kernel<SPLIT><<<grid, C::NUM_THREADS, C::SMEM_BYTES, st>>>(p, q, w3h, w3l, w1h, w1l, tres, tout, r1h, r1l, st32);
  return check_launch("conv_chain_tc_kernel");
}

}

extern "C" int hd_conv_gemm_chain_supported(const hd_conv_desc *first, const hd_conv_desc *second) {
  return hd::chain_check(first, second) == HD_OK ? 1 : 0;
}

extern "C" int hd_conv_gemm_chain(const hd_conv_desc *first, const hd_conv_desc *second, void *stream) {
  int rc = hd::chain_check(first, second);
  if (rc) return rc;
  hd::ConvParams p, q;
  if ((rc = hd::fill_params(first, p))) return rc;
  hd_conv_desc b = *second;
  b.in_hi = first->in_hi;
  b.in_lo = first->in_lo;
  if ((rc = hd::fill_params(&b, q))) return rc;
  if (!p.vec_out || !q.vec_out) {
    hd::set_last_error_text("hd_conv_gemm_chain: outputs and epilogue vectors must be 16-byte aligned");
    return HD_ERR_INVALID;
  }
  cudaStream_t st = (cudaStream_t)stream;
  return first->impl == HD_IMPL_TC_3XF16 ? hd::launch_chain<true>(p, q, first, second, st) : hd::launch_chain<false>(p, q, first, second, st);
}

extern "C" int hd_make_weight_tmap(const void *w_nk, int rows, int k_pad, int box_rows, int elem_bytes, void *tmap_out) {
  HD_REQUIRE(w_nk && tmap_out && rows > 0 && k_pad > 0 && (elem_bytes == 4 || elem_bytes == 2) && k_pad % (128 / elem_bytes) == 0 &&
                 box_rows == 64 && rows % box_rows == 0 && hd::aligned16(w_nk),
             "hd_make_weight_tmap: bad arguments");
  hd::EncodeTiledFn fn = hd::get_encode_fn();
  if (!fn) { hd::set_last_error_text("cuTensorMapEncodeTiled unavailable (no CUDA driver?)"); return HD_ERR_UNSUPPORTED; }
  alignas(64) CUtensorMap tm;
  const cuuint64_t gdim[2] = {(cuuint64_t)k_pad, (cuuint64_t)rows};
  const cuuint64_t gstride[1] = {(cuuint64_t)k_pad * (cuuint64_t)elem_bytes};
  const cuuint32_t box[2] = {(cuuint32_t)(128 / elem_bytes), (cuuint32_t)box_rows};
  const cuuint32_t estr[2] = {1u, 1u};
  CUresult r = fn(&tm, elem_bytes == 4 ? CU_TENSOR_MAP_DATA_TYPE_FLOAT32 : CU_TENSOR_MAP_DATA_TYPE_FLOAT16, 2, const_cast<void *>(w_nk),
                  gdim, gstride, box, estr, CU_TENSOR_MAP_INTERLEAVE_NONE, CU_TENSOR_MAP_SWIZZLE_128B,
                  CU_TENSOR_MAP_L2_PROMOTION_L2_128B, CU_TENSOR_MAP_FLOAT_OOB_FILL_NONE);
  if (r != CUDA_SUCCESS) {
    char msg[96];
    snprintf(msg, sizeof(msg), "cuTensorMapEncodeTiled failed with CUresult %d", (int)r);
    hd::set_last_error_text(msg);
    return HD_ERR_CUDA;
  }
  memcpy(tmap_out, &tm, sizeof(tm));
  return HD_OK;
}

extern "C" int hd_make_act_tmap(const void *base, long long rows, int cols, long long ld_elems, int elem_bytes, void *tmap_out) {
  HD_REQUIRE(base && tmap_out && rows > 0 && cols > 0 && ld_elems >= cols && (elem_bytes == 4 || elem_bytes == 2) && hd::aligned16(base) &&
                 (ld_elems * elem_bytes) % 16 == 0,
             "hd_make_act_tmap: bad arguments (16-byte aligned base and row pitch required)");
  hd::EncodeTiledFn fn = hd::get_encode_fn();
  if (!fn) { hd::set_last_error_text("cuTensorMapEncodeTiled unavailable (no CUDA driver?)"); return HD_ERR_UNSUPPORTED; }
  alignas(64) CUtensorMap tm;
  const cuuint64_t gdim[2] = {(cuuint64_t)cols, (cuuint64_t)rows};
  const cuuint64_t gstride[1] = {(cuuint64_t)ld_elems * (cuuint64_t)elem_bytes};
  const cuuint32_t box[2] = {32u, 128u};
  const cuuint32_t estr[2] = {1u, 1u};
  CUresult r = fn(&tm, elem_bytes == 4 ? CU_TENSOR_MAP_DATA_TYPE_FLOAT32 : CU_TENSOR_MAP_DATA_TYPE_FLOAT16, 2, const_cast<void *>(base), gdim,
                  gstride, box, estr, CU_TENSOR_MAP_INTERLEAVE_NONE, elem_bytes == 4 ? CU_TENSOR_MAP_SWIZZLE_128B : CU_TENSOR_MAP_SWIZZLE_64B,
                  CU_TENSOR_MAP_L2_PROMOTION_L2_128B, CU_TENSOR_MAP_FLOAT_OOB_FILL_NONE);
  if (r != CUDA_SUCCESS) {
    char msg[96];
    snprintf(msg, sizeof(msg), "cuTensorMapEncodeTiled (activation) failed with CUresult %d", (int)r);
    hd::set_last_error_text(msg);
    return HD_ERR_CUDA;
  }
  memcpy(tmap_out, &tm, sizeof(tm));
  return HD_OK;
}
```

human_dynamics_b200/csrc/tc_ptx.cuh:

```cuda
#pragma once
#include <cuda.h>
#include <cuda_fp16.h>
#include <stdint.h>

namespace hd {
namespace ptx {

static __device__ __forceinline__ uint32_t smem_u32(const void *p) { return (uint32_t)__cvta_generic_to_shared(p); }

static __device__ __forceinline__ void mbar_init(uint32_t bar, uint32_t count) {
  asm volatile("mbarrier.init.shared::cta.b64 [%0], %1;" ::"r"(bar), "r"(count) : "memory");
}
static __device__ __forceinline__ void mbar_arrive(uint32_t bar) {
  asm volatile("mbarrier.arrive.shared::cta.b64 _, [%0];" ::"r"(bar) : "memory");
}
static __device__ __forceinline__ void mbar_arrive_expect_tx(uint32_t bar, uint32_t bytes) {
  asm volatile("mbarrier.arrive.expect_tx.shared::cta.b64 _, [%0], %1;" ::"r"(bar), "r"(bytes) : "memory");
}
static __device__ __forceinline__ void mbar_wait(uint32_t bar, uint32_t parity) {
  uint32_t done;
  do {
    asm volatile(
        "{\n.reg .pred p;\nmbarrier.try_wait.parity.shared::cta.b64 p, [%1], %2;\nselp.u32 %0, 1, 0, p;\n}"
        : "=r"(done)
        : "r"(bar), "r"(parity)
        : "memory");
  } while (!done);
}
static __device__ __forceinline__ void tma_load_2d(uint32_t dst, const CUtensorMap *tmap, uint32_t bar, int c0, int c1) {
  asm volatile(
      "cp.async.bulk.tensor.2d.shared::cluster.global.mbarrier::complete_tx::bytes [%0], [%1, {%3, %4}], [%2];" ::"r"(dst),
      "l"(reinterpret_cast<uint64_t>(tmap)), "r"(bar), "r"(c0), "r"(c1)
      : "memory");
}
static __device__ __forceinline__ void tma_store_2d(const CUtensorMap *tmap, uint32_t src, int c0, int c1) {
  asm volatile("cp.async.bulk.tensor.2d.global.shared::cta.bulk_group [%0, {%2, %3}], [%1];" ::"l"(reinterpret_cast<uint64_t>(tmap)),
               "r"(src), "r"(c0), "r"(c1)
               : "memory");
}
static __device__ __forceinline__ void tma_prefetch_2d(const CUtensorMap *tmap, int c0, int c1) {
  asm volatile("cp.async.bulk.prefetch.tensor.2d.L2.global [%0, {%1, %2}];" ::"l"(reinterpret_cast<uint64_t>(tmap)), "r"(c0), "r"(c1)
               : "memory");
}
static __device__ __forceinline__ void bulk_commit() { asm volatile("cp.async.bulk.commit_group;" ::: "memory"); }
template <int N>
static __device__ __forceinline__ void bulk_wait_read() { asm volatile("cp.async.bulk.wait_group.read %0;" ::"n"(N) : "memory"); }
static __device__ __forceinline__ void bulk_wait_all() { asm volatile("cp.async.bulk.wait_group 0;" ::: "memory"); }
static __device__ __forceinline__ void fence_proxy_async() { asm volatile("fence.proxy.async.shared::cta;" ::: "memory"); }
static __device__ __forceinline__ void named_bar_sync(int id, int threads) { asm volatile("bar.sync %0, %1;" ::"r"(id), "r"(threads) : "memory"); }
static __device__ __forceinline__ bool elect_one() {
  uint32_t pred;
  asm volatile("{\n.reg .pred p;\nelect.sync _|p, 0xffffffff;\nselp.u32 %0, 1, 0, p;\n}" : "=r"(pred));
  return pred != 0;
}
static __device__ __forceinline__ void cp_async16(uint32_t dst, const void *src, uint32_t src_bytes) {
  asm volatile("cp.async.cg.shared.global [%0], [%1], 16, %2;" ::"r"(dst), "l"(src), "r"(src_bytes) : "memory");
}
static __device__ __forceinline__ void cp_async16_ca(uint32_t dst, const void *src, uint32_t src_bytes) {
  asm volatile("cp.async.ca.shared.global [%0], [%1], 16, %2;" ::"r"(dst), "l"(src), "r"(src_bytes) : "memory");
}
static __device__ __forceinline__ void cp_async_commit() { asm volatile("cp.async.commit_group;" ::: "memory"); }
template <int N>
static __device__ __forceinline__ void cp_async_wait() { asm volatile("cp.async.wait_group %0;" ::"n"(N) : "memory"); }

static __device__ __forceinline__ float rn_tf32(float x) { return __uint_as_float((__float_as_uint(x) + 0x1000u) & 0xFFFFE000u); }

static __device__ __forceinline__ void wgmma_fence() { asm volatile("wgmma.fence.sync.aligned;" ::: "memory"); }
static __device__ __forceinline__ void wgmma_commit() { asm volatile("wgmma.commit_group.sync.aligned;" ::: "memory"); }
template <int N>
static __device__ __forceinline__ void wgmma_wait() { asm volatile("wgmma.wait_group.sync.aligned %0;" ::"n"(N) : "memory"); }
template <int R>
static __device__ __forceinline__ void fence_regs(float (&d)[R]) {
#pragma unroll
  for (int i = 0; i < R; ++i) asm volatile("" : "+f"(d[i])::"memory");
}
static __device__ __forceinline__ void wgmma_m64n64k16_f16(float (&d)[32], uint64_t da, uint64_t db, uint32_t scale_d) {
  asm volatile(
      "{\n.reg .pred p;\nsetp.ne.b32 p, %34, 0;\n"
      "wgmma.mma_async.sync.aligned.m64n64k16.f32.f16.f16 "
      "{%0, %1, %2, %3, %4, %5, %6, %7, %8, %9, %10, %11, %12, %13, %14, %15, %16, %17, %18, %19, %20, %21, %22, %23, %24, %25, %26, %27, %28, %29, %30, %31}, "
      "%32, %33, p, 1, 1, 0, 0;\n}\n"
      : "+f"(d[0]), "+f"(d[1]), "+f"(d[2]), "+f"(d[3]), "+f"(d[4]), "+f"(d[5]), "+f"(d[6]), "+f"(d[7]), "+f"(d[8]), "+f"(d[9]), "+f"(d[10]), "+f"(d[11]), "+f"(d[12]), "+f"(d[13]), "+f"(d[14]), "+f"(d[15]), "+f"(d[16]), "+f"(d[17]), "+f"(d[18]), "+f"(d[19]), "+f"(d[20]), "+f"(d[21]), "+f"(d[22]), "+f"(d[23]), "+f"(d[24]), "+f"(d[25]), "+f"(d[26]), "+f"(d[27]), "+f"(d[28]), "+f"(d[29]), "+f"(d[30]), "+f"(d[31])
      : "l"(da), "l"(db), "r"(scale_d));
}
static __device__ __forceinline__ void wgmma_m64n64k8_tf32(float (&d)[32], uint64_t da, uint64_t db, uint32_t scale_d) {
  asm volatile(
      "{\n.reg .pred p;\nsetp.ne.b32 p, %34, 0;\n"
      "wgmma.mma_async.sync.aligned.m64n64k8.f32.tf32.tf32 "
      "{%0, %1, %2, %3, %4, %5, %6, %7, %8, %9, %10, %11, %12, %13, %14, %15, %16, %17, %18, %19, %20, %21, %22, %23, %24, %25, %26, %27, %28, %29, %30, %31}, "
      "%32, %33, p, 1, 1;\n}\n"
      : "+f"(d[0]), "+f"(d[1]), "+f"(d[2]), "+f"(d[3]), "+f"(d[4]), "+f"(d[5]), "+f"(d[6]), "+f"(d[7]), "+f"(d[8]), "+f"(d[9]), "+f"(d[10]), "+f"(d[11]), "+f"(d[12]), "+f"(d[13]), "+f"(d[14]), "+f"(d[15]), "+f"(d[16]), "+f"(d[17]), "+f"(d[18]), "+f"(d[19]), "+f"(d[20]), "+f"(d[21]), "+f"(d[22]), "+f"(d[23]), "+f"(d[24]), "+f"(d[25]), "+f"(d[26]), "+f"(d[27]), "+f"(d[28]), "+f"(d[29]), "+f"(d[30]), "+f"(d[31])
      : "l"(da), "l"(db), "r"(scale_d));
}
static __device__ __forceinline__ void wgmma_m64n128k16_f16(float (&d)[64], uint64_t da, uint64_t db, uint32_t scale_d) {
  asm volatile(
      "{\n.reg .pred p;\nsetp.ne.b32 p, %66, 0;\n"
      "wgmma.mma_async.sync.aligned.m64n128k16.f32.f16.f16 "
      "{%0, %1, %2, %3, %4, %5, %6, %7, %8, %9, %10, %11, %12, %13, %14, %15, %16, %17, %18, %19, %20, %21, %22, %23, %24, %25, %26, %27, %28, %29, %30, %31, %32, %33, %34, %35, %36, %37, %38, %39, %40, %41, %42, %43, %44, %45, %46, %47, %48, %49, %50, %51, %52, %53, %54, %55, %56, %57, %58, %59, %60, %61, %62, %63}, "
      "%64, %65, p, 1, 1, 0, 0;\n}\n"
      : "+f"(d[0]), "+f"(d[1]), "+f"(d[2]), "+f"(d[3]), "+f"(d[4]), "+f"(d[5]), "+f"(d[6]), "+f"(d[7]), "+f"(d[8]), "+f"(d[9]), "+f"(d[10]), "+f"(d[11]), "+f"(d[12]), "+f"(d[13]), "+f"(d[14]), "+f"(d[15]), "+f"(d[16]), "+f"(d[17]), "+f"(d[18]), "+f"(d[19]), "+f"(d[20]), "+f"(d[21]), "+f"(d[22]), "+f"(d[23]), "+f"(d[24]), "+f"(d[25]), "+f"(d[26]), "+f"(d[27]), "+f"(d[28]), "+f"(d[29]), "+f"(d[30]), "+f"(d[31]), "+f"(d[32]), "+f"(d[33]), "+f"(d[34]), "+f"(d[35]), "+f"(d[36]), "+f"(d[37]), "+f"(d[38]), "+f"(d[39]), "+f"(d[40]), "+f"(d[41]), "+f"(d[42]), "+f"(d[43]), "+f"(d[44]), "+f"(d[45]), "+f"(d[46]), "+f"(d[47]), "+f"(d[48]), "+f"(d[49]), "+f"(d[50]), "+f"(d[51]), "+f"(d[52]), "+f"(d[53]), "+f"(d[54]), "+f"(d[55]), "+f"(d[56]), "+f"(d[57]), "+f"(d[58]), "+f"(d[59]), "+f"(d[60]), "+f"(d[61]), "+f"(d[62]), "+f"(d[63])
      : "l"(da), "l"(db), "r"(scale_d));
}
static __device__ __forceinline__ void wgmma_m64n256k16_f16(float (&d)[128], uint64_t da, uint64_t db, uint32_t scale_d) {
  asm volatile(
      "{\n.reg .pred p;\nsetp.ne.b32 p, %130, 0;\n"
      "wgmma.mma_async.sync.aligned.m64n256k16.f32.f16.f16 "
      "{%0, %1, %2, %3, %4, %5, %6, %7, %8, %9, %10, %11, %12, %13, %14, %15, %16, %17, %18, %19, %20, %21, %22, %23, %24, %25, %26, %27, %28, %29, %30, %31, %32, %33, %34, %35, %36, %37, %38, %39, %40, %41, %42, %43, %44, %45, %46, %47, %48, %49, %50, %51, %52, %53, %54, %55, %56, %57, %58, %59, %60, %61, %62, %63, %64, %65, %66, %67, %68, %69, %70, %71, %72, %73, %74, %75, %76, %77, %78, %79, %80, %81, %82, %83, %84, %85, %86, %87, %88, %89, %90, %91, %92, %93, %94, %95, %96, %97, %98, %99, %100, %101, %102, %103, %104, %105, %106, %107, %108, %109, %110, %111, %112, %113, %114, %115, %116, %117, %118, %119, %120, %121, %122, %123, %124, %125, %126, %127}, "
      "%128, %129, p, 1, 1, 0, 0;\n}\n"
      : "+f"(d[0]), "+f"(d[1]), "+f"(d[2]), "+f"(d[3]), "+f"(d[4]), "+f"(d[5]), "+f"(d[6]), "+f"(d[7]), "+f"(d[8]), "+f"(d[9]), "+f"(d[10]), "+f"(d[11]), "+f"(d[12]), "+f"(d[13]), "+f"(d[14]), "+f"(d[15]), "+f"(d[16]), "+f"(d[17]), "+f"(d[18]), "+f"(d[19]), "+f"(d[20]), "+f"(d[21]), "+f"(d[22]), "+f"(d[23]), "+f"(d[24]), "+f"(d[25]), "+f"(d[26]), "+f"(d[27]), "+f"(d[28]), "+f"(d[29]), "+f"(d[30]), "+f"(d[31]), "+f"(d[32]), "+f"(d[33]), "+f"(d[34]), "+f"(d[35]), "+f"(d[36]), "+f"(d[37]), "+f"(d[38]), "+f"(d[39]), "+f"(d[40]), "+f"(d[41]), "+f"(d[42]), "+f"(d[43]), "+f"(d[44]), "+f"(d[45]), "+f"(d[46]), "+f"(d[47]), "+f"(d[48]), "+f"(d[49]), "+f"(d[50]), "+f"(d[51]), "+f"(d[52]), "+f"(d[53]), "+f"(d[54]), "+f"(d[55]), "+f"(d[56]), "+f"(d[57]), "+f"(d[58]), "+f"(d[59]), "+f"(d[60]), "+f"(d[61]), "+f"(d[62]), "+f"(d[63]), "+f"(d[64]), "+f"(d[65]), "+f"(d[66]), "+f"(d[67]), "+f"(d[68]), "+f"(d[69]), "+f"(d[70]), "+f"(d[71]), "+f"(d[72]), "+f"(d[73]), "+f"(d[74]), "+f"(d[75]), "+f"(d[76]), "+f"(d[77]), "+f"(d[78]), "+f"(d[79]), "+f"(d[80]), "+f"(d[81]), "+f"(d[82]), "+f"(d[83]), "+f"(d[84]), "+f"(d[85]), "+f"(d[86]), "+f"(d[87]), "+f"(d[88]), "+f"(d[89]), "+f"(d[90]), "+f"(d[91]), "+f"(d[92]), "+f"(d[93]), "+f"(d[94]), "+f"(d[95]), "+f"(d[96]), "+f"(d[97]), "+f"(d[98]), "+f"(d[99]), "+f"(d[100]), "+f"(d[101]), "+f"(d[102]), "+f"(d[103]), "+f"(d[104]), "+f"(d[105]), "+f"(d[106]), "+f"(d[107]), "+f"(d[108]), "+f"(d[109]), "+f"(d[110]), "+f"(d[111]), "+f"(d[112]), "+f"(d[113]), "+f"(d[114]), "+f"(d[115]), "+f"(d[116]), "+f"(d[117]), "+f"(d[118]), "+f"(d[119]), "+f"(d[120]), "+f"(d[121]), "+f"(d[122]), "+f"(d[123]), "+f"(d[124]), "+f"(d[125]), "+f"(d[126]), "+f"(d[127])
      : "l"(da), "l"(db), "r"(scale_d));
}

static __device__ __forceinline__ uint64_t make_smem_desc(uint32_t saddr) {
  uint64_t d = 0;
  d |= (uint64_t)((saddr & 0x3FFFFu) >> 4);
  d |= (uint64_t)1 << 16;
  d |= (uint64_t)(1024 >> 4) << 32;
  d |= (uint64_t)1 << 62;
  return d;
}


}
}
```

include/hd_b200.h:

```cpp
#ifndef HD_B200_H_
#define HD_B200_H_

#include <stddef.h>
#include <stdint.h>

#ifdef __cplusplus
extern "C" {
#endif

typedef enum {
  HD_OK = 0,
  HD_ERR_INVALID = 1,
  HD_ERR_WORKSPACE = 2,
  HD_ERR_CUDA = 3,
  HD_ERR_UNSUPPORTED = 4
} hd_status;

int hd_version(void);
const char *hd_status_string(int status);
const char *hd_last_error(void);
long long hd_launch_count(void);
void hd_launch_count_reset(void);

enum { HD_IMPL_SIMT = 0, HD_IMPL_TC_3XTF32 = 1, HD_IMPL_TC_1XTF32 = 2, HD_IMPL_TC_3XF16 = 3, HD_IMPL_TC_1XF16 = 4 };

typedef struct {
  const float *in;  long long in_ld;
  int n_img, H, W, Cin;
  int Ho, Wo, KH, KW, stride, pad_t, pad_l;
  const float *w_kn;
  const void *w_nk_hi;
  const void *w_nk_lo;
  int Cout;  int K_pad;
  const float *pre_scale, *pre_shift;  int pre_img_stride;  int pre_relu;
  const float *post_scale, *post_shift;  int post_relu;
  const float *res;  long long res_ld;  int res_H, res_W, res_stride;
  float *out;  long long out_ld;
  int impl;
  const void *tmap_hi, *tmap_lo;
  const void *in_hi, *in_lo;
  void *out_hi, *out_lo;  long long out2_ld;
  const float *post2_scale, *post2_shift;  int post2_relu;
  const void *tmap_res, *tmap_out, *tmap_out_hi, *tmap_out_lo;
  int flags;
  const void *tmap_hi_n64, *tmap_lo_n64;
  int out_subsample;
} hd_conv_desc;

enum {
  HD_CONV_NO_TMA_EPILOGUE = 1,
  HD_CONV_INPUT_PLANES = 2
};

int hd_conv_gemm(const hd_conv_desc *d, void *stream);
int hd_conv_gemm_profile(const hd_conv_desc *d, void *stream, long long *dbg);
int hd_conv_gemm_chain(const hd_conv_desc *first, const hd_conv_desc *second, void *stream);
int hd_conv_gemm_chain_supported(const hd_conv_desc *first, const hd_conv_desc *second);

int hd_make_weight_tmap(const void *w_nk, int rows, int k_pad, int box_rows, int elem_bytes, void *tmap_out);
int hd_make_act_tmap(const void *base, long long rows, int cols, long long ld_elems, int elem_bytes, void *tmap_out);

int hd_pack_conv1_planes(const float *img, void *plane_hi, void *plane_lo, int N, int H, int W, int WP, void *stream);
int hd_conv1_7x7s2(const float *in, const float *w, const float *bias, float *out, int N, int H, int W, void *stream);
int hd_maxpool3x3s2_same(const float *in, float *out, int N, int H, int W, int C, const float *scale, const float *shift,
                         void *out_hi, void *out_lo, void *stream);
int hd_subsample(const float *in, float *out, int N, int H, int W, int C, int stride, void *stream);
int hd_bnrelu_avgpool(const float *in, const float *scale, const float *shift, float *out, int N, int HW, int C, void *stream);

size_t hd_bn_stats_workspace_bytes(long long rows, int C);
int hd_bn_batch_stats(const float *x, long long rows, int C, long long ld, const float *gamma, const float *beta, float eps,
                      float *scale, float *shift, float *mean, float *var, float *moving_mean, float *moving_var, double decay,
                      void *workspace, size_t workspace_bytes, void *stream);
int hd_bn_moving_update(const float *mean, const float *var, long long rows, int C, double decay, float *moving_mean, float *moving_var,
                        void *stream);

size_t hd_conv_wgrad_workspace_bytes(long long pixels, int K, int Cout, int bias);
int hd_conv_wgrad(const float *x, long long x_ld, int n_img, int H, int W, int Cin, int Ho, int Wo, int KH, int KW, int stride, int pad_t,
                  int pad_l, const float *pre_scale, const float *pre_shift, const float *dy, long long dy_ld, int Cout, float *dw, float *db,
                  void *workspace, size_t workspace_bytes, void *stream);
int hd_conv_wgrad_ex(const float *x, long long x_ld, int n_img, int H, int W, int Cin, int Ho, int Wo, int KH, int KW, int stride, int pad_t,
                     int pad_l, const float *pre_scale, const float *pre_shift, const float *dy, long long dy_ld, int Cout, float *dw,
                     float *db, void *workspace, size_t workspace_bytes, int impl, void *stream);
size_t hd_bn_relu_backward_workspace_bytes(long long rows, int C);
int hd_bn_relu_backward(const float *x, const float *dz, int dz_group, long long rows, int C, const float *scale, const float *shift,
                        const float *var, const float *gamma, float eps, const float *addend, int add_H, int add_W, int add_stride,
                        float *dx, float *dgamma, float *dbeta, void *workspace, size_t workspace_bytes, void *stream);
int hd_maxpool3x3s2_same_backward(const float *in, const float *dout, float *din, int N, int H, int W, int C, void *stream);
int hd_zero_insert(const float *in, float *out, int N, int Hi, int Wi, int C, int stride, int Ho, int Wo, void *stream);

int hd_process_image(const unsigned char *frames, int N, int H, int W, const int *geom, float *out, int S, void *plane_hi,
                     void *plane_lo, int WP, void *stream);
int hd_crop_geometry(int H, int W, const double *bbox, int img_size, int *geom, int *center, int *start_pt);

#define HD_AUG_SRC_U8 1
#define HD_AUG_ROTATE 2
#define HD_AUG_FLIP 4
typedef struct {
  const void *frames;
  int F, H, W, flags;
  const int *trans;
  const float *scale, *rot;
  const int *flip;
  const float *labels;
  int K;
  const int *centers;
  const float *poses, *gt3ds;
  int S, trans_max;
  int *geom;
  float *labels_out;
  int *centers_out;
  float *poses_out, *gt3ds_out;
  float *crops;
  void *plane_hi, *plane_lo;
  int WP;
} hd_tube_aug_args;
int hd_tube_augment(const hd_tube_aug_args *a, void *stream);

int hd_groupnorm_stats(const float *x, const float *gamma, const float *beta, float *gain, float *offset,
                       int B, int T, int C, int groups, float eps, void *stream);

int hd_groupnorm_relu_split(const float *x, const float *gamma, const float *beta, void *out_hi, void *out_lo, int B, int T, int C,
                            int groups, float eps, void *stream);
int hd_split_f16(const float *x, void *hi, void *lo, long long n, void *stream);

int hd_ief_fc1_theta(const float *P, const float *theta, int theta_ld, const float *W, int K, int C, void *out_hi, void *out_lo,
                     float *out_f32, int N, void *stream);
int hd_ief_fc3(const float *h2, const float *W, const float *bias, const float *prev, int prev_ld, float *out, int out_ld, int N, int K,
               int D, void *stream);

int hd_ief_fc1_theta_dropout(const float *P, const float *theta, int theta_ld, const float *W, int K, int C, void *out_hi, void *out_lo,
                             float *out_f32, int N, unsigned long long seed, unsigned long long step, int site, float p, void *stream);
int hd_ief_fc3_dropout(float *h2, const float *W, const float *bias, const float *prev, int prev_ld, float *out, int out_ld, int N, int K,
                       int D, unsigned long long seed, unsigned long long step, int site, float p, void *stream);
int hd_dropout_mask(unsigned long long seed, unsigned long long step, int site, int N, int C, float p, unsigned char *out, void *stream);

int hd_ief_delta_init(const float *theta, float *dst, int dst_ld, int N, void *stream);

typedef struct hd_net hd_net;
typedef const float *(*hd_weight_fn)(void *user, const char *tf_name, long long *numel);
void hd_net_destroy(hd_net *net);
const char *hd_net_error(const hd_net *net);
long long hd_net_num_launches(const hd_net *net);
int hd_resnet50_create(hd_weight_fn get, void *user, int n_frames, int size, hd_net **net);
int hd_resnet50_forward(hd_net *net, const float *images, float *phi, void *stream);
int hd_fmovie_create(hd_weight_fn get, void *user, int B, int T, int num_conv_layers, hd_net **net);
int hd_fmovie_forward(hd_net *net, const float *phi, float *out, void *stream);
int hd_ief_create(hd_weight_fn get, void *user, int N, const int *delta_t, int num_delta, hd_net **net);
int hd_ief_forward(hd_net *net, const float *phi, float *theta, float *deltas, void *stream);

typedef struct {
  int num_verts, num_kps, lbs_nnz, kp_nnz_total;
  const float *v_template;
  const float *dirs;
  const float *J_template;
  const float *J_shapedirs;
  const int *lbs_idx;
  const float *lbs_w;
  const int *kp_ptr;
  const int *kp_vidx;
  const float *kp_w;
  int parents[24];
} hd_smpl_consts;

int hd_smpl_pack_sizes(int V, int K, const double *weights, const double *kp_regressor, int *lbs_nnz, int *kp_nnz_total);
int hd_smpl_pack(int V, int K, const double *v_template, const double *shapedirs, const double *posedirs, const double *J_regressor,
                 const double *weights, const double *kp_regressor, const unsigned int *kintree_parents, float *v_template_out, float *dirs,
                 float *J_template, float *J_shapedirs, int *lbs_idx, float *lbs_w, int lbs_nnz, int *kp_ptr, int *kp_vidx, float *kp_w,
                 int *parents);
size_t hd_smpl_workspace_bytes(int N);
int hd_smpl_forward(const hd_smpl_consts *c, const float *beta, int beta_ld, const float *theta, int theta_ld, int N,
                    float *verts, float *joints, float *Rs, float *Jtr,
                    const float *cam, int cam_ld, float *kps, int out_mul, int out_off,
                    void *ws, size_t ws_bytes, void *stream);
int hd_smpl_pose(const hd_smpl_consts *c, const float *beta, int beta_ld, const float *theta, int theta_ld, int N, float *Rs,
                 float *Jtr, float *A12, float *coef , int coef_ld,
                 void *coef_hi, void *coef_lo ,
                 void *a12t_hi, void *a12t_lo ,
                 int out_mul, int out_off, void *ws, size_t ws_bytes, void *stream);
int hd_smpl_lbs_tc(const void *w_hi, const void *w_lo, const void *a12t_hi, const void *a12t_lo, const float *v_posed, long long vp_ld,
                   float *verts, int N, int V, int out_mul, int out_off, void *stream);
int hd_smpl_lbs(const hd_smpl_consts *c, const float *v_posed, long long vp_ld, const float *A12, float *verts, int N, int out_mul,
                int out_off, void *stream);
int hd_smpl_joints(const hd_smpl_consts *c, const float *verts, const float *cam, int cam_ld, float *joints, float *kps, int N,
                   int out_mul, int out_off, void *stream);
int hd_rodrigues(const float *theta, float *R, int M, void *stream);
int hd_rot2aa(const float *Rs, float *aa, int M, void *stream);
int hd_global_rigid(const float *Rs, const float *Js, const int *parents_host, float *new_J, float *A44, int N,
                    int rotate_base, void *stream);
int hd_orth_proj(const float *X, const float *cam, float *out, int N, int P, void *stream);

enum { HD_SMPL_GRAD_TILE = 256, HD_SMPL_GRAD_CLD = 224 };
typedef struct {
  int num_verts, num_kps, num_tiles, tile_verts;
  const int *kpv_ptr;
  const int *kpv_kidx;
  const float *kpv_w;
  const int *lbt_ptr;
  const int *lbt_v;
  const float *lbt_w;
} hd_smpl_grad_consts;
size_t hd_smpl_backward_workspace_bytes(int N, int V);
int hd_smpl_lbs_backward(const hd_smpl_consts *c, const hd_smpl_grad_consts *g, const float *v_posed, long long vp_ld, const float *A12,
                         const float *dverts, const float *djoints, float *dv_posed, float *dA12, int N, void *stream);
int hd_smpl_pose_backward(const hd_smpl_consts *c, const float *beta, int beta_ld, const float *theta, int theta_ld, int N,
                          const float *dA12, const float *dc, int dc_ld, const float *dRs, const float *dJtr, float *dbeta, int dbeta_ld,
                          float *dtheta, int dtheta_ld, void *stream);
int hd_rodrigues_backward(const float *theta, const float *dR, float *dtheta, int M, void *stream);
int hd_global_rigid_backward(const float *Rs, const float *Js, const int *parents_host, const float *dnew_J, const float *dA44, float *dRs,
                             float *dJs, int N, int rotate_base, void *stream);
int hd_orth_proj_backward(const float *X, const float *cam, const float *dout, float *dX, float *dcam, int N, int P, void *stream);

enum { HD_PACK_FORWARD = 0, HD_PACK_BACKWARD_DATA = 1 };
int hd_pack_weight(const float *w, int KH, int Cin, int Cout, int mode, int elem_bytes, void *hi, void *lo, int rows, int k_pad, void *stream);
int hd_transpose_split(const float *x, long long rows, int cols, long long ld, int mode, void *hi, void *lo, long long out_ld, int out_rows,
                       long long out_cols, void *stream);
int hd_im2col_t(const float *x, int B, int T, int C, int KH, int pad, const float *gain, const float *offset, int relu, float *out,
                long long out_ld, long long out_cols, void *stream);
int hd_groupnorm_relu_backward(const float *x, const float *gamma, const float *beta, const float *dy, const float *addend, float *dx,
                               float *dgamma_part, float *dbeta_part, int B, int T, int C, int groups, float eps, int relu, void *stream);
int hd_col_sum(const float *x, long long rows, int cols, long long ld, float *out, void *stream);
int hd_relu_backward(const float *y, const float *dy, float *dx, long long n, void *stream);
int hd_relu_dropout_backward(const float *y, const float *dy, float *dx, long long n, float p, void *stream);
int hd_fc_small_dgrad(const float *g, int g_ld, const float *Wt, int K, int D, const float *mask, float *out, int N, void *stream);
int hd_fc_small_dgrad_dropout(const float *g, int g_ld, const float *Wt, int K, int D, const float *mask, float p, float *out, int N,
                              void *stream);
int hd_add_strided(const float *a, long long lda, const float *b, long long ldb, float *out, long long ldo, int rows, int cols, void *stream);

enum { HD_DPOSE_JOINTS = 23, HD_DPOSE_GRAD_FLOATS = 3160 };
size_t hd_dpose_workspace_bytes(int N);
int hd_dpose_trunk_forward(const float *x, const float *W1, const float *b1, const float *W2, const float *b2, const float *wj,
                           const float *bj, float *h1, float *h2, float *logits, int N, void *stream);
int hd_dpose_out_forward(const float *h, const float *w_out, const float *b_out, float *logits, int N, void *stream);
int hd_dpose_trunk_backward(const float *x, const float *h1, const float *h2, const float *dflat, const float *g, const float *hf,
                            const float *W1, const float *W2, const float *wj, float *dx, void *ws, size_t ws_bytes, int N, void *stream);
int hd_dpose_grad_reduce(const void *ws, size_t ws_bytes, int N, float *grad, void *stream);

enum { HD_LOSS_KP_L1 = 0, HD_LOSS_MSE_ROWS = 1 };
enum { HD_LOSS_KP_CAMERA = 0, HD_LOSS_KP_OPTCAM = 1, HD_LOSS_KP_RAW = 2 };
enum { HD_LOSS_MAX_TERMS = 64, HD_LOSS_MAX_GRADS = 16 };
typedef struct {
  int kind, proj;
  int B, Tw, p_t0, q_t0, p_T, q_T;
  int K, D;
  const float *p;
  long long p_clip, p_frame;
  const float *q;
  long long q_clip, q_frame;
  const float *cam;
  long long cam_clip, cam_frame;
  const float *w;
  float *cam_out;
  float scale;
} hd_loss_term;
typedef struct {
  const float *src;
  float *grad;
  long long numel;
} hd_loss_grad;
size_t hd_loss_workspace_bytes(const hd_loss_term *terms, int n);
int hd_loss_forward(const hd_loss_term *terms, int n, float *values, void *ws, size_t ws_bytes, void *stream);
int hd_loss_backward(const hd_loss_term *terms, int n, const hd_loss_grad *grads, int n_grads, const float *dvalues, const void *ws,
                     size_t ws_bytes, void *stream);

enum { HD_ADAM_MAX_TENSORS = 256 };
typedef struct {
  float *param;
  const float *grad;
  float *m;
  float *v;
  long long numel;
} hd_adam_tensor;
int hd_adam_tf(const hd_adam_tensor *t, int n, float lr, float beta1, float beta2, float epsilon, float *powers, void *stream);

typedef struct {
  float color[3], light_dir[3], ambient, directional, bg[3], near_z, far_z, eye_z;
  float rot[9];
  int use_rot;
} hd_render_params;
size_t hd_render_workspace_bytes(int N, int S, int F);
int hd_render_mesh(const float *verts, long long verts_ld, int N, int V, const int *faces, int F, const float *cam, int cam_ld,
                   const hd_render_params *p, const float *background , int S,
                   unsigned char *out_rgb , float *out_alpha , void *ws, size_t ws_bytes,
                   void *stream);

enum { HD_EVAL_KP = 0, HD_EVAL_KP_PA = 1, HD_EVAL_KP_PCK = 2, HD_EVAL_JOINTS = 3, HD_EVAL_JOINTS_PA = 4, HD_EVAL_ACCEL = 5,
       HD_EVAL_ACCEL_ERROR = 6, HD_EVAL_VIS3D = 7, HD_EVAL_COLS = 8 };
typedef struct {
  int N, n_seq;
  const int *seq_start;
  int K, J;
  const float *kps_gt;
  long long kps_gt_ld;
  const float *kps_pred;
  long long kps_pred_ld;
  const float *joints_gt;
  long long joints_gt_ld;
  const float *joints_pred;
  long long joints_pred_ld;
  float img_size;
  int min_visible;
  double *out;
} hd_eval_frames_args;
int hd_eval_frames(const hd_eval_frames_args *a, void *stream);
int hd_eval_mesh_tpose(const hd_smpl_consts *c, const float *beta_gt, int beta_gt_ld, const float *beta_pred, int beta_pred_ld, int N,
                       double *out, void *stream);
int hd_eval_verts_error(const float *a, long long a_ld, const float *b, long long b_ld, int N, int V, double *out, void *stream);

enum { HD_JPEG_BAD_CODE = 1, HD_JPEG_OVERRUN = 2, HD_JPEG_MARKER = 4, HD_JPEG_BAD_HEADER = 8 };
typedef struct {
  uint8_t bits[16];
  uint8_t vals[256];
} hd_jpeg_huffman;
typedef struct {
  int width, height;
  int h_samp, v_samp;
  int restart_interval;
  int qt[3], dc[3], ac[3];
  long long data_offset, data_bytes;
} hd_jpeg_header;
typedef struct {
  uint16_t quant[4][64];
  hd_jpeg_huffman dc[4], ac[4];
  int quant_defined, dc_defined, ac_defined;
} hd_jpeg_tables;
int hd_jpeg_parse(const uint8_t *data, size_t len, hd_jpeg_header *hdr, hd_jpeg_tables *tables);
size_t hd_jpeg_workspace_bytes(int N, int H, int W, int h_samp, int v_samp);
int hd_jpeg_decode(const uint8_t *data, long long data_size, const hd_jpeg_header *hdrs, int N, int H, int W, int h_samp, int v_samp,
                   const uint16_t *quant, int n_quant, const hd_jpeg_huffman *huff, int n_huff, uint8_t *out, int *status,
                   void *workspace, size_t workspace_bytes, void *stream);

#ifdef __cplusplus
}
#endif
#endif
```

Before: 14760.

## Add ping-pong 64x128 tile variant for deep-K 1x1 pre-split convolutions

Adds a ping-pong mode to the warp-specialized wgmma conv kernel. The two consumer warpgroups take alternate 64-row tiles and hand off through named barriers, so one group's epilogue overlaps the other's MMA mainloop. Tile selection is refactored to route 1x1 layers with K a multiple of 128 to this variant when the wide-N heuristic favours it, and a query API reporting the chosen tile is added. The cost is more template instantiations, plus possible stalls from the barrier handoff and from smaller M tiles.

```diff
diff --git a/human_dynamics_b200/_lib.py b/human_dynamics_b200/_lib.py
--- a/human_dynamics_b200/_lib.py
+++ b/human_dynamics_b200/_lib.py
@@ -154,6 +154,7 @@
     'hd_conv_gemm_profile': (_i, [C.POINTER(ConvDesc), _vp, _vp]),
     'hd_conv_gemm_chain': (_i, [C.POINTER(ConvDesc), C.POINTER(ConvDesc), _vp]),
     'hd_conv_gemm_chain_supported': (_i, [C.POINTER(ConvDesc), C.POINTER(ConvDesc)]),
+    'hd_conv_gemm_tile': (_i, [C.POINTER(ConvDesc), _i, _vp]),
     'hd_make_weight_tmap': (_i, [_vp, _i, _i, _i, _i, _vp]),
     'hd_make_act_tmap': (_i, [_vp, _ll, _i, _ll, _i, _vp]),
     'hd_pack_conv1_planes': (_i, [_vp, _vp, _vp, _i, _i, _i, _i, _vp]),
diff --git a/human_dynamics_b200/csrc/conv_tc.cu b/human_dynamics_b200/csrc/conv_tc.cu
--- a/human_dynamics_b200/csrc/conv_tc.cu
+++ b/human_dynamics_b200/csrc/conv_tc.cu
@@ -14,14 +14,15 @@
 
 using namespace ptx;
 
-template <bool SPLIT, bool HALF, bool ASPLIT, int BN, bool RES = false, bool SHORT = false, bool CM = false>
+template <bool SPLIT, bool HALF, bool ASPLIT, int BN, bool RES = false, bool SHORT = false, bool CM = false, bool PP = false>
 struct Cfg {
   static_assert(BN == 64 || (BN == 128 && HALF && ASPLIT), "128-wide N tiles: pre-split fp16 path only");
   static_assert(!RES || ASPLIT, "residual by TMA: pre-split fp16 path only");
   static_assert(!SHORT || (BN == 64 && HALF && ASPLIT), "two CTAs per SM: 64-wide pre-split fp16 tiles only");
   static_assert(!CM || (BN == 64 && HALF && ASPLIT && !RES && !SHORT), "channels on M: 64-channel pre-split fp16 tiles, no residual");
+  static_assert(!PP || (BN == 128 && !SHORT && !CM), "ping-pong: 64 x 128 pre-split tiles");
   static constexpr int CTAS = SHORT ? 2 : 1;
-  static constexpr int TM = CM ? 256 : BM;
+  static constexpr int TM = CM ? 256 : PP ? 64 : BM;
   static constexpr int A_BYTES = TM * 128;
   static constexpr int PROD_THREADS = BN == 128 || SHORT || CM ? 128 : 256;
   static constexpr int NUM_THREADS = 256 + PROD_THREADS;
@@ -31,7 +32,7 @@
   static_assert(256 * CONS_REGS + PROD_THREADS * PROD_REGS <= NUM_THREADS * (65536 / (CTAS * NUM_THREADS) / 8 * 8),
                 "setmaxnreg split beyond the CTA's registers");
   static constexpr int NACC = CM ? 64 : BN / 2;
-  static constexpr int STAGES = SHORT ? 1 : CM ? 2 : BN == 128 ? (RES ? 2 : 3) : (RES ? 3 : 4);
+  static constexpr int STAGES = SHORT ? 1 : CM ? 2 : PP ? (RES ? 2 : 4) : BN == 128 ? (RES ? 2 : 3) : (RES ? 3 : 4);
   static constexpr int BKE = HALF ? 64 : 32;
   static constexpr int B_TILE_BYTES = BN * 128;
   static constexpr int B_OFFSET = (SPLIT ? 2 : 1) * A_BYTES;
@@ -63,12 +64,12 @@
   int n[R], iy[R], ix[R];
 };
 
-template <bool SPLIT, int PCH, bool HALF, bool GATHER, bool ASPLIT, int BN, bool RES, bool SHORT, bool CM>
-__global__ void __launch_bounds__((Cfg<SPLIT, HALF, ASPLIT, BN, RES, SHORT, CM>::NUM_THREADS), (Cfg<SPLIT, HALF, ASPLIT, BN, RES, SHORT, CM>::CTAS))
+template <bool SPLIT, int PCH, bool HALF, bool GATHER, bool ASPLIT, int BN, bool RES, bool SHORT, bool CM, bool PP>
+__global__ void __launch_bounds__((Cfg<SPLIT, HALF, ASPLIT, BN, RES, SHORT, CM, PP>::NUM_THREADS), (Cfg<SPLIT, HALF, ASPLIT, BN, RES, SHORT, CM, PP>::CTAS))
 conv_gemm_tc_kernel(const ConvParams p, const __grid_constant__ CUtensorMap tmap_hi, const __grid_constant__ CUtensorMap tmap_lo,
                     const __grid_constant__ CUtensorMap tmap_res, const __grid_constant__ CUtensorMap tmap_out,
                     const __grid_constant__ CUtensorMap tmap_out_hi, const __grid_constant__ CUtensorMap tmap_out_lo, const int stage) {
-  using C = Cfg<SPLIT, HALF, ASPLIT, BN, RES, SHORT, CM>;
+  using C = Cfg<SPLIT, HALF, ASPLIT, BN, RES, SHORT, CM, PP>;
   constexpr bool MEM_STAMPS = BN == 128 || SHORT || CM;
   constexpr int BKE = C::BKE, PF = C::PF, V = C::V, STAGES = C::STAGES, R = C::ROWS, RS = C::ROW_STEP, NA = C::NACC;
   extern __shared__ uint8_t smem_raw[];
@@ -88,7 +89,7 @@
   if (threadIdx.x == 0) {
     for (int s = 0; s < STAGES; ++s) {
       mbar_init(full_bar(s), ASPLIT ? C::PROD_THREADS + 1 : 9);
-      mbar_init(empty_bar(s), 8);
+      mbar_init(empty_bar(s), PP ? 4 : 8);
     }
     if (RES) for (int g = 0; g < 2; ++g) mbar_init(res_bar(g), 1);
     asm volatile("fence.mbarrier_init.release.cluster;" ::: "memory");
@@ -144,7 +145,7 @@
     if constexpr (ASPLIT) {
       const __half *ihi = reinterpret_cast<const __half *>(p.in_hi);
       const __half *ilo = reinterpret_cast<const __half *>(p.in_lo);
-      if (SHORT || (!CM && !p.planes && p.KH * p.KW <= 32 && (long long)p.n_img * p.H * p.W * p.in_ld < (1ll << 31))) {
+      if (SHORT || PP || (!CM && !p.planes && p.KH * p.KW <= 32 && (long long)p.n_img * p.H * p.W * p.in_ld < (1ll << 31))) {
         const uint32_t off0 = (uint32_t)rb * 128u + sw_off;
         int base[R];
         uint32_t mask[R];
@@ -197,7 +198,7 @@
           }
           if (++kc == num_k) { kc = 0; ++ti; }
         }
-      } else if (!SHORT && p.planes && (long long)p.n_img * p.H * p.W * p.in_ld < (1ll << 31)) {
+      } else if (!SHORT && !PP && p.planes && (long long)p.n_img * p.H * p.W * p.in_ld < (1ll << 31)) {
         const uint32_t off0 = (uint32_t)rb * 128u + sw_off;
         const int jt = j >> 2;
         const int row_step = 2 * p.W * (int)p.in_ld;
@@ -238,7 +239,7 @@
           asm volatile("cp.async.mbarrier.arrive.noinc.shared::cta.b64 [%0];" ::"r"(full_bar(s)) : "memory");
           if (++kc == num_k) { kc = 0; ++ti; }
         }
-      } else if (!SHORT && !CM) {
+      } else if (!SHORT && !CM && !PP) {
       RowState<R> rs;
       int kc = 0, ti = 0;
       for (int q = 0; q < total; ++q) {
@@ -400,12 +401,13 @@
   } else if (warp < W_PROD) {
     asm volatile("setmaxnreg.inc.sync.aligned.u32 %0;" ::"n"(C::CONS_REGS));
     const int wg = warp >> 2;
+    const int rw = PP ? 0 : wg;
     const bool prof = p.dbg != nullptr && blockIdx.x == 0 && threadIdx.x == 0;
     long long t_wait = 0, t_start = prof && !MEM_STAMPS && !RES ? clock64() : 0;
     if ((RES || MEM_STAMPS) && prof) p.dbg[2] = clock64();
-    if (prof) { p.dbg[3] = 0; p.dbg[4] = 0; p.dbg[5] = 0; p.dbg[6] = 0; }
+    if (prof) { p.dbg[3] = 0; p.dbg[4] = 0; p.dbg[5] = 0; p.dbg[6] = 0; p.dbg[9] = 0; }
     const int hw = p.Ho * p.Wo;
-    const int frow = wg * 64 + (warp & 3) * 16 + (lane >> 2);
+    const int frow = rw * 64 + (warp & 3) * 16 + (lane >> 2);
     const int fcol = 2 * (lane & 3);
     float acc[NA], accx[SPLIT ? NA : 1], sums_[SHORT ? 1 : NA];
     float *const sums = SHORT ? acc : sums_;
@@ -419,20 +421,70 @@
     const bool stg_issuer = ASPLIT && (threadIdx.x & 127) == 0;
     auto load_res = [&](int ti) {
       const int tile = (int)blockIdx.x + ti * (int)gridDim.x;
-      const int r0 = (tile / tiles_n) * BM + 64 * wg, c0 = (tile % tiles_n) * BN;
+      const int r0 = (tile / tiles_n) * C::TM + 64 * rw, c0 = (tile % tiles_n) * BN;
       const int cols = p.Cout - c0 < BN ? p.Cout - c0 : BN;
       const int boxes = r0 < p.M ? (cols + 31) / 32 : 0;
       const uint32_t slot = smem_base + C::RES_OFFSET + wg * C::RES_SLOT_BYTES;
       mbar_arrive_expect_tx(res_bar(wg), boxes * (64 * 128));
       for (int b = 0; b < boxes; ++b) tma_load_2d(slot + b * (64 * 128), &tmap_res, res_bar(wg), c0 + 32 * b, r0);
     };
-    if (res_issuer && my_tiles > 0) load_res(0);
-    int q = 0;
-    for (int ti = 0; ti < my_tiles; ++ti) {
+    constexpr int TSTEP = PP ? 2 : 1;
+    const int ti0 = PP ? wg : 0;
+    if (res_issuer && ti0 < my_tiles) load_res(ti0);
+    for (int ti = ti0; ti < my_tiles; ti += TSTEP) {
       if (!SHORT) {
 #pragma unroll
         for (int i = 0; i < NA; ++i) sums[i] = 0.f;
       }
+      if (PP && ti > 0) {
+        if (prof) p.dbg[9] -= clock64();
+        named_bar_sync(5 + wg, 256);
+        if (prof) p.dbg[9] += clock64();
+      }
+      int q = ti * num_k;
+      if constexpr (PP) {
+        static_assert(!PP || PCH == 2, "ping-pong: flush groups of two chunks");
+        for (int kc = 0; kc < num_k; kc += 2, q += 2) {
+          long long tw = 0;
+#pragma unroll
+          for (int u = 0; u < 2; ++u) {
+            const int s = (q + u) % STAGES;
+            const long long t0 = clock64();
+            mbar_wait(full_bar(s), (uint32_t)((q + u) / STAGES) & 1u);
+            tw += clock64() - t0;
+            asm volatile("fence.proxy.async.shared::cta;" ::: "memory");
+            const uint32_t a_hi = smem_base + s * C::STAGE_BYTES, b_hi = a_hi + C::B_OFFSET;
+            const uint64_t da_hi = make_smem_desc(a_hi), da_lo = make_smem_desc(a_hi + C::A_BYTES);
+            const uint64_t db_hi = make_smem_desc(b_hi), db_lo = make_smem_desc(b_hi + C::B_TILE_BYTES);
+            if (u == 0) {
+              fence_regs(acc);
+              if constexpr (SPLIT) fence_regs(accx);
+            }
+            wgmma_fence();
+#pragma unroll
+            for (int k = 0; k < 4; ++k) {
+              const uint64_t adv = (uint64_t)((k * 32) >> 4);
+              if constexpr (SPLIT) {
+                wgmma_m64n128k16_f16(accx, da_lo + adv, db_hi + adv, ((kc + u) | k) != 0);
+                wgmma_m64n128k16_f16(accx, da_hi + adv, db_lo + adv, 1u);
+              }
+              wgmma_m64n128k16_f16(acc, da_hi + adv, db_hi + adv, !(u == 0 && k == 0));
+            }
+            wgmma_commit();
+          }
+          wgmma_wait<1>();
+          __syncwarp();
+          if (lane == 0) mbar_arrive(empty_bar(q % STAGES));
+          wgmma_wait<0>();
+          fence_regs(acc);
+          if constexpr (SPLIT) fence_regs(accx);
+          __syncwarp();
+          if (lane == 0) mbar_arrive(empty_bar((q + 1) % STAGES));
+          if (prof) p.dbg[3] += tw;
+#pragma unroll
+          for (int i = 0; i < NA; ++i) sums[i] += acc[i];
+        }
+      } else
       for (int kc = 0; kc < num_k; ++kc, ++q) {
         const int s = q % STAGES;
         const uint32_t ph = (uint32_t)(q / STAGES) & 1u;
@@ -443,7 +495,7 @@
         if (!MEM_STAMPS && prof) t_wait += clock64() - tw0;
         if (MEM_STAMPS && prof) p.dbg[3] += clock64();
         if (ASPLIT) asm volatile("fence.proxy.async.shared::cta;" ::: "memory");
-        const uint32_t a_hi = smem_base + s * C::STAGE_BYTES + wg * (C::TM / 2 * 128);
+        const uint32_t a_hi = smem_base + s * C::STAGE_BYTES + rw * (C::TM / 2 * 128);
         const uint32_t a_lo = a_hi + C::A_BYTES;
         const uint32_t b_hi = smem_base + s * C::STAGE_BYTES + C::B_OFFSET;
         const uint32_t b_lo = b_hi + C::B_TILE_BYTES;
@@ -492,6 +544,7 @@
           for (int i = 0; i < NA; ++i) sums[i] += acc[i];
         }
       }
+      if (PP && ti + 1 < my_tiles) named_bar_arrive(5 + (wg ^ 1), 256);
       if (SHORT) {
 #pragma unroll
         for (int i = 0; i < NA; ++i) acc[i] = __fadd_rn(0.f, acc[i]);
@@ -504,7 +557,7 @@
       const int tile = (int)blockIdx.x + ti * (int)gridDim.x;
       const int m0 = (tile / tiles_n) * C::TM, n0 = (tile % tiles_n) * BN;
       if (RES && prof) p.dbg[5] -= clock64();
-      if (RES) mbar_wait(res_bar(wg), (uint32_t)ti & 1u);
+      if (RES) mbar_wait(res_bar(wg), (uint32_t)(ti / TSTEP) & 1u);
       if (RES && prof) p.dbg[5] += clock64();
       auto row_geom = [&](int m, int &n_img, int &oy, int &ox) {
         n_img = 0; oy = 0; ox = 0;
@@ -587,7 +640,7 @@
         const bool st32 = (stage & STAGE_OUT) != 0, st2 = (stage & STAGE_PAIR) != 0;
         uint8_t *stg = smem + C::STG_OFFSET + wg * C::STG_BYTES;
         const uint32_t stg_a = smem_base + C::STG_OFFSET + wg * C::STG_BYTES;
-        const int r0 = m0 + 64 * wg;
+        const int r0 = m0 + 64 * rw;
         const uint32_t rsw = (uint32_t)(lane >> 2);
         auto acquire = [&](bool after_out) {
           if (prof) p.dbg[6] -= clock64();
@@ -606,7 +659,7 @@
           const bool rok[2] = {m0 + frow < p.M, m0 + frow + 8 < p.M};
           if (!RES && !st32 && st2 && !p.out && !p.res) {
             acquire(false);
-            uint8_t *brow = stg + (frow - 64 * wg) * 128 + 4 * (lane & 3);
+            uint8_t *brow = stg + (frow - 64 * rw) * 128 + 4 * (lane & 3);
             const float *vsc = p.post_scale ? p.post_scale + c0 + fcol : nullptr, *vsh = p.post_shift ? p.post_shift + c0 + fcol : nullptr;
             const float *v2sc = p.post2_scale ? p.post2_scale + c0 + fcol : nullptr, *v2sh = p.post2_shift ? p.post2_shift + c0 + fcol : nullptr;
 #pragma unroll
@@ -640,7 +693,7 @@
             continue;
           }
           if (st32 && (RES || !p.res)) {
-            uint8_t *brow = (RES ? res_sm + 2 * cc * BOX_BYTES : stg) + (frow - 64 * wg) * 128 + 8 * (lane & 1);
+            uint8_t *brow = (RES ? res_sm + 2 * cc * BOX_BYTES : stg) + (frow - 64 * rw) * 128 + 8 * (lane & 1);
             const float *vsc = p.post_scale ? p.post_scale + c0 + fcol : nullptr, *vsh = p.post_shift ? p.post_shift + c0 + fcol : nullptr;
 #pragma unroll
             for (int jj = 0; jj < 8; ++jj) {
@@ -668,7 +721,7 @@
             row_geom(m, n_img, oy, ox);
             const float *rrow = res_row(m, n_img, oy, ox);
             float *orow = st32 ? nullptr : out_row(m, n_img, oy, ox);
-            uint8_t *brow = (RES ? res_sm + 2 * cc * BOX_BYTES : stg) + (frow - 64 * wg + 8 * h) * 128 + 8 * (lane & 1);
+            uint8_t *brow = (RES ? res_sm + 2 * cc * BOX_BYTES : stg) + (frow - 64 * rw + 8 * h) * 128 + 8 * (lane & 1);
 #pragma unroll
             for (int jj = 0; jj < 8; ++jj) {
               const int j = 8 * cc + jj;
@@ -697,7 +750,7 @@
           if (p.out_hi) {
             if (st2) acquire(RES && st32 && !SHORT);
             if (st2) {
-              uint8_t *brow = stg + (frow - 64 * wg) * 128 + 4 * (lane & 3);
+              uint8_t *brow = stg + (frow - 64 * rw) * 128 + 4 * (lane & 3);
               const float *vsc = p.post2_scale ? p.post2_scale + c0 + fcol : nullptr, *vsh = p.post2_shift ? p.post2_shift + c0 + fcol : nullptr;
 #pragma unroll
               for (int jj = 0; jj < 8; ++jj) {
@@ -724,7 +777,7 @@
               if (m >= p.M) continue;
               __half *hrow = reinterpret_cast<__half *>(p.out_hi) + (size_t)m * p.out2_ld;
               __half *lrow = SPLIT ? reinterpret_cast<__half *>(p.out_lo) + (size_t)m * p.out2_ld : nullptr;
-              uint8_t *brow = stg + (frow - 64 * wg + 8 * h) * 128 + 4 * (lane & 3);
+              uint8_t *brow = stg + (frow - 64 * rw + 8 * h) * 128 + 4 * (lane & 3);
 #pragma unroll
               for (int jj = 0; jj < 8; ++jj) {
                 const int j = 8 * cc + jj;
@@ -795,7 +848,7 @@
         }
       }
       }
-      if (RES && ti + 1 < my_tiles) {
+      if (RES && ti + TSTEP < my_tiles) {
         if (prof) p.dbg[6] -= clock64();
         named_bar_sync(1 + wg, 128);
         if (res_issuer) {
@@ -805,7 +858,7 @@
             if (stage & STAGE_PAIR) bulk_wait_read<1>();
             else bulk_wait_read<0>();
           }
-          load_res(ti + 1);
+          load_res(ti + TSTEP);
         }
         if (prof) p.dbg[6] += clock64();
       }
@@ -1140,16 +1193,16 @@
 }
 
 template <bool SPLIT, int PCH, bool HALF, bool GATHER = false, bool ASPLIT = false, int BN = 64, bool RES = false, bool SHORT = false,
-          bool CM = false>
+          bool CM = false, bool PP = false>
 int launch_tc(const ConvParams &p, const hd_conv_desc *d, cudaStream_t st) {
-  using C = Cfg<SPLIT, HALF, ASPLIT, BN, RES, SHORT, CM>;
+  using C = Cfg<SPLIT, HALF, ASPLIT, BN, RES, SHORT, CM, PP>;
   static bool configured[kMaxDevices] = {};
   static int num_sms[kMaxDevices] = {};
   int dev = 0;
   cudaGetDevice(&dev);
   if (dev < 0 || dev >= kMaxDevices) { set_last_error_text("conv_gemm_tc: device ordinal out of range"); return HD_ERR_UNSUPPORTED; }
   if (!configured[dev]) {
-    cudaError_t e = cudaFuncSetAttribute(conv_gemm_tc_kernel<SPLIT, PCH, HALF, GATHER, ASPLIT, BN, RES, SHORT, CM>,
+    cudaError_t e = cudaFuncSetAttribute(conv_gemm_tc_kernel<SPLIT, PCH, HALF, GATHER, ASPLIT, BN, RES, SHORT, CM, PP>,
                                          cudaFuncAttributeMaxDynamicSharedMemorySize, C::SMEM_BYTES);
     if (e != cudaSuccess) { set_last_error("conv_gemm_tc attr", e); return HD_ERR_CUDA; }
     cudaDeviceGetAttribute(&num_sms[dev], cudaDevAttrMultiProcessorCount, dev);
@@ -1182,29 +1235,46 @@
   const int num_tiles = ceil_div(p.M, C::TM) * ceil_div(p.Cout, BN);
   const int ctas = C::CTAS * num_sms[dev];
   dim3 grid(num_tiles < ctas ? num_tiles : ctas);
-  conv_gemm_tc_kernel<SPLIT, PCH, HALF, GATHER, ASPLIT, BN, RES, SHORT, CM>
+  conv_gemm_tc_kernel<SPLIT, PCH, HALF, GATHER, ASPLIT, BN, RES, SHORT, CM, PP>
       <<<grid, C::NUM_THREADS, C::SMEM_BYTES, st>>>(p, thi, tlo, tres, tout, tohi, tolo, stage);
   return check_launch("conv_gemm_tc_kernel");
 }
 
-bool wide_n_tile(const ConvParams &p) {
-  if (p.Cout <= 64) return false;
+int device_sms() {
   int dev = 0, sms = 0;
   cudaGetDevice(&dev);
   cudaDeviceGetAttribute(&sms, cudaDevAttrMultiProcessorCount, dev);
+  return sms;
+}
+
+bool wide_n_tile(const ConvParams &p, int tm, int sms) {
+  if (p.Cout <= 64) return false;
   if (sms <= 0) return true;
-  const long long m_tiles = ceil_div(p.M, BM);
-  const long long w128 = (m_tiles * ceil_div(p.Cout, 128) + sms - 1) / sms, w64 = (m_tiles * ceil_div(p.Cout, 64) + sms - 1) / sms;
-  return 16 * w128 <= 9 * w64;
+  const long long wide = (ceil_div(p.M, tm) * ceil_div(p.Cout, 128) + sms - 1) / sms;
+  const long long w64 = (ceil_div(p.M, BM) * ceil_div(p.Cout, 64) + sms - 1) / sms;
+  return 8 * (tm / 64) * wide <= 9 * w64;
+}
+
+enum PreSplitTile { TILE_128x64, TILE_128x128, TILE_64x128_PP, TILE_SHORT };
+
+bool res_rows_layer(const ConvParams &p) {
+  return p.res && p.res_stride == 1 && p.res_H == p.Ho && p.res_W == p.Wo && p.K <= 8 * 64;
+}
+
+PreSplitTile pre_split_tile(const ConvParams &p, int sms, bool short_two_ctas) {
+  const bool lean_1x1 = p.KH * p.KW == 1 && (long long)p.n_img * p.H * p.W * p.in_ld < (1ll << 31);
+  const bool short_k = p.K <= 2 * 64 && lean_1x1 && (p.res ? res_rows_layer(p) : p.out_hi != nullptr);
+  if (short_k && short_two_ctas) return TILE_SHORT;
+  const bool pingpong = p.K > 2 * 64 && p.K % (2 * 64) == 0 && lean_1x1;
+  if (wide_n_tile(p, pingpong ? 64 : BM, sms)) return pingpong ? TILE_64x128_PP : TILE_128x128;
+  return TILE_128x64;
 }
 
 
 bool cout_on_m(const ConvParams &p) {
   if (!p.planes || p.Cout != 64 || p.res || p.out_sub || p.out_hi || !p.out) return false;
   if ((long long)p.n_img * p.H * p.W * p.in_ld >= (1ll << 31)) return false;
-  int dev = 0, sms = 0;
-  cudaGetDevice(&dev);
-  cudaDeviceGetAttribute(&sms, cudaDevAttrMultiProcessorCount, dev);
+  const int sms = device_sms();
   if (sms <= 0) return true;
   const long long w256 = (ceil_div(p.M, 256) + sms - 1) / sms, w128 = (ceil_div(p.M, BM) + sms - 1) / sms;
   return 16 * w256 <= 9 * w128;
@@ -1218,7 +1288,7 @@
   cudaGetDevice(&dev);
   if (dev < 0 || dev >= kMaxDevices) return false;
   if (two[dev] == 0) {
-    const auto kernel = conv_gemm_tc_kernel<SPLIT, 2, true, false, true, 64, RES, true, false>;
+    const auto kernel = conv_gemm_tc_kernel<SPLIT, 2, true, false, true, 64, RES, true, false, false>;
     int n = 0;
     if (cudaFuncSetAttribute(kernel, cudaFuncAttributeMaxDynamicSharedMemorySize, C::SMEM_BYTES) != cudaSuccess ||
         cudaOccupancyMaxActiveBlocksPerMultiprocessor(&n, kernel, C::NUM_THREADS, C::SMEM_BYTES) != cudaSuccess) {
@@ -1245,15 +1315,19 @@
       set_last_error_text("hd_conv_gemm(tc split-A): needs Cin % 64 == 0, in_ld % 8 == 0, aligned in_hi/in_lo, no prologue");
       return HD_ERR_INVALID;
     }
-    const bool res_rows = p.res && p.res_stride == 1 && p.res_H == p.Ho && p.res_W == p.Wo && p.K <= 8 * 64;
-    const bool short_k = p.K <= 2 * 64 && p.KH * p.KW == 1 && (long long)p.n_img * p.H * p.W * p.in_ld < (1ll << 31) &&
-                         (p.res ? res_rows : p.out_hi != nullptr);
-    if (short_k && (res_rows ? short_k_two_ctas<SPLIT, true>() : short_k_two_ctas<SPLIT, false>()))
-      return res_rows ? launch_tc<SPLIT, 2, true, false, true, 64, true, true>(p, d, st)
-                      : launch_tc<SPLIT, 2, true, false, true, 64, false, true>(p, d, st);
-    if (wide_n_tile(p))
-      return res_rows ? launch_tc<SPLIT, 2, true, false, true, 128, true>(p, d, st) : launch_tc<SPLIT, 2, true, false, true, 128>(p, d, st);
-    return res_rows ? launch_tc<SPLIT, 2, true, false, true, 64, true>(p, d, st) : launch_tc<SPLIT, 2, true, false, true>(p, d, st);
+    const bool res_rows = res_rows_layer(p);
+    switch (pre_split_tile(p, device_sms(), res_rows ? short_k_two_ctas<SPLIT, true>() : short_k_two_ctas<SPLIT, false>())) {
+      case TILE_SHORT:
+        return res_rows ? launch_tc<SPLIT, 2, true, false, true, 64, true, true>(p, d, st)
+                        : launch_tc<SPLIT, 2, true, false, true, 64, false, true>(p, d, st);
+      case TILE_64x128_PP:
+        return res_rows ? launch_tc<SPLIT, 2, true, false, true, 128, true, false, false, true>(p, d, st)
+                        : launch_tc<SPLIT, 2, true, false, true, 128, false, false, false, true>(p, d, st);
+      case TILE_128x128:
+        return res_rows ? launch_tc<SPLIT, 2, true, false, true, 128, true>(p, d, st) : launch_tc<SPLIT, 2, true, false, true, 128>(p, d, st);
+      default:
+        return res_rows ? launch_tc<SPLIT, 2, true, false, true, 64, true>(p, d, st) : launch_tc<SPLIT, 2, true, false, true>(p, d, st);
+    }
   }
   if (p.Cin % 64 != 0) {
     const int segp = (p.KW * p.Cin + 7) & ~7;
@@ -1375,6 +1449,20 @@
   return hd::chain_check(first, second) == HD_OK ? 1 : 0;
 }
 
+extern "C" int hd_conv_gemm_tile(const hd_conv_desc *d, int num_sms, int *tile) {
+  HD_REQUIRE(d && tile && num_sms > 0, "hd_conv_gemm_tile: bad arguments");
+  hd::ConvParams p;
+  if (int rc = hd::fill_params(d, p)) return rc;
+  if ((d->impl != HD_IMPL_TC_3XF16 && d->impl != HD_IMPL_TC_1XF16) || !p.in_hi || p.planes) {
+    hd::set_last_error_text("hd_conv_gemm_tile: pre-split layers of impl 3 / 4 only");
+    return HD_ERR_UNSUPPORTED;
+  }
+  static const int shapes[4][4] = {{128, 64, 1, 0}, {128, 128, 1, 0}, {64, 128, 1, 1}, {128, 64, 2, 0}};
+  const int *s = shapes[hd::pre_split_tile(p, num_sms, true)];
+  for (int i = 0; i < 4; ++i) tile[i] = s[i];
+  return HD_OK;
+}
+
 extern "C" int hd_conv_gemm_chain(const hd_conv_desc *first, const hd_conv_desc *second, void *stream) {
   int rc = hd::chain_check(first, second);
   if (rc) return rc;
diff --git a/human_dynamics_b200/csrc/tc_ptx.cuh b/human_dynamics_b200/csrc/tc_ptx.cuh
--- a/human_dynamics_b200/csrc/tc_ptx.cuh
+++ b/human_dynamics_b200/csrc/tc_ptx.cuh
@@ -48,6 +48,7 @@
 static __device__ __forceinline__ void bulk_wait_all() { asm volatile("cp.async.bulk.wait_group 0;" ::: "memory"); }
 static __device__ __forceinline__ void fence_proxy_async() { asm volatile("fence.proxy.async.shared::cta;" ::: "memory"); }
 static __device__ __forceinline__ void named_bar_sync(int id, int threads) { asm volatile("bar.sync %0, %1;" ::"r"(id), "r"(threads) : "memory"); }
+static __device__ __forceinline__ void named_bar_arrive(int id, int threads) { asm volatile("bar.arrive %0, %1;" ::"r"(id), "r"(threads) : "memory"); }
 static __device__ __forceinline__ bool elect_one() {
   uint32_t pred;
   asm volatile("{\n.reg .pred p;\nelect.sync _|p, 0xffffffff;\nselp.u32 %0, 1, 0, p;\n}" : "=r"(pred));
diff --git a/include/hd_b200.h b/include/hd_b200.h
--- a/include/hd_b200.h
+++ b/include/hd_b200.h
@@ -56,6 +56,7 @@
 int hd_conv_gemm_profile(const hd_conv_desc *d, void *stream, long long *dbg);
 int hd_conv_gemm_chain(const hd_conv_desc *first, const hd_conv_desc *second, void *stream);
 int hd_conv_gemm_chain_supported(const hd_conv_desc *first, const hd_conv_desc *second);
+int hd_conv_gemm_tile(const hd_conv_desc *d, int num_sms, int *tile);
 
 int hd_make_weight_tmap(const void *w_nk, int rows, int k_pad, int box_rows, int elem_bytes, void *tmap_out);
 int hd_make_act_tmap(const void *base, long long rows, int cols, long long ld_elems, int elem_bytes, void *tmap_out);
```

Result: no change. 14680, median of 6 (-0.6%).
